# EAST-J/Dynhor

Hardware: AMD Instinct MI355X
Metric: training rays/sec (higher is better)
Workload: dtype f32; 1 GPU; custom_shoes-shaped synthetic seq, 512x512, 2048 rays x (64+64) samples per rank, NeuS SDF(8x256, skip 4, softplus100) + colour(4x256) MLP, full training iteration; family=neus, frames=64, rays_per_rank=2048, samples_per_ray=128, parallelism=dp1, loss=rgb L1 + 0.1 eikonal + 0.1 mask BCE + 0.05 mono-normal

## Files before the change

### dynhor_amd/_lib.py

```python
import ctypes
import os

import torch

_HERE = os.path.dirname(os.path.abspath(__file__))
LIB_PATH = os.path.join(_HERE, "libdynhor_hip.so")
_LIB = None

_vp, _i64, _i32, _f32 = ctypes.c_void_p, ctypes.c_int64, ctypes.c_int, ctypes.c_float

SIGNATURES = {
    "dh_version": (_i32, []),
    "dh_strerror": (ctypes.c_char_p, [_i32]),
    "dh_set_arithmetic": (_i32, [_i32]),
    "dh_get_arithmetic": (_i32, []),
    "dh_hash_set_scatter_mode": (_i32, [_i32]),
    "dh_num_params": (_i64, []),
    "dh_packed_floats": (_i64, []),
    "dh_param_layout": (_i32, [_i32, _i32, ctypes.POINTER(_i64), ctypes.POINTER(_i64), ctypes.POINTER(_i64),
                               ctypes.POINTER(_i32), ctypes.POINTER(_i32)]),
    "dh_packed_section": (_i32, [_i32, ctypes.POINTER(_i64), ctypes.POINTER(_i64)]),
    "dh_pack_weights": (_i32, [_vp, _vp, _vp]),
    "dh_pack_weights_ex": (_i32, [_i32, _vp, _vp, _vp]),
    "dh_sdf_nograd": (_i32, [_vp, _vp, _i64, _vp, _vp]),
    "dh_workspace_floats": (_i32, [_i64, ctypes.POINTER(_i64), ctypes.POINTER(_i64), ctypes.POINTER(_i64)]),
    "dh_range_words": (_i32, [ctypes.POINTER(_i64), ctypes.POINTER(_i64), ctypes.POINTER(_f32)]),
    "dh_mlp_forward": (_i32, [_vp, _vp, _vp, _i32, _i64, _vp, _vp, _vp, _vp, _vp]),
    "dh_sdf_forward": (_i32, [_vp, _vp, _i64, _vp, _vp, _vp]),
    "dh_sdf_gradient": (_i32, [_vp, _vp, _i64, _vp, _vp, _i32, _vp]),
    "dh_color_forward": (_i32, [_vp, _vp, _vp, _i32, _vp, _i64, _vp, _vp, _i32, _vp]),
    "dh_color_backward": (_i32, [_vp, _vp, _vp, _i64, _vp, _vp, _vp]),
    "dh_sdf_tangent": (_i32, [_vp, _vp, _vp, _i64, _vp, _vp]),
    "dh_sdf_backward": (_i32, [_vp, _vp, _i64, _vp, _vp]),
    "dh_color_backward_rays": (_i32, [_vp, _vp, _vp, _vp, _i32, _i64, _vp, _vp, _vp, _vp, _vp]),
    "dh_sdf_backward_rays": (_i32, [_vp, _vp, _vp, _vp, _i64, _vp, _vp, _vp]),
    "dh_weight_grads_gemm": (_i32, [_i64, _vp, _vp]),
    "dh_weight_grads_fold": (_i32, [_vp, _vp, _i64, _vp, _vp, _vp]),
    "dh_mlp_backward": (_i32, [_vp, _vp, _vp, _i64] + [_vp] * 7),
    "dh_sdf_nograd_ex": (_i32, [_i32, _vp, _vp, _i64, _vp, _vp]),
    "dh_mlp_forward_ex": (_i32, [_i32, _vp, _vp, _vp, _i32, _i64, _vp, _vp, _vp, _vp, _vp]),
    "dh_sdf_forward_ex": (_i32, [_i32, _vp, _vp, _i64, _vp, _vp, _vp]),
    "dh_sdf_gradient_ex": (_i32, [_i32, _vp, _vp, _i64, _vp, _vp, _i32, _vp]),
    "dh_color_forward_ex": (_i32, [_i32, _vp, _vp, _vp, _i32, _vp, _i64, _vp, _vp, _i32, _vp]),
    "dh_color_backward_ex": (_i32, [_i32, _vp, _vp, _vp, _i64, _vp, _vp, _vp]),
    "dh_sdf_tangent_ex": (_i32, [_i32, _vp, _vp, _vp, _i64, _vp, _vp]),
    "dh_sdf_backward_ex": (_i32, [_i32, _vp, _vp, _i64, _vp, _vp]),
    "dh_color_backward_rays_ex": (_i32, [_i32, _vp, _vp, _vp, _vp, _i32, _i64, _vp, _vp, _vp, _vp, _vp]),
    "dh_sdf_backward_rays_ex": (_i32, [_i32, _vp, _vp, _vp, _vp, _i64, _vp, _vp, _vp]),
    "dh_weight_grads_gemm_ex": (_i32, [_i32, _i64, _vp, _vp]),
    "dh_mlp_backward_ex": (_i32, [_i32, _vp, _vp, _vp, _i64] + [_vp] * 7),
    "dh_adam_step": (_i32, [_vp, _vp, _vp, _vp, _i64, _f32, _f32, _f32, _f32, _i64, _f32, _vp]),
    "dh_hashgrid_entries": (_i64, []),
    "dh_hashgrid_level": (_i32, [_i32, ctypes.POINTER(_f32), ctypes.POINTER(ctypes.c_uint32), ctypes.POINTER(ctypes.c_uint32),
                                 ctypes.POINTER(ctypes.c_uint32)]),
    "dh_hashgrid_encode": (_i32, [_vp, _vp, _i64, _vp, _vp]),
    "dh_hashgrid_encode_backward": (_i32, [_vp, _vp, _i64, _vp, _vp]),
    "dh_hash_num_params": (_i64, []),
    "dh_hash_packed_floats": (_i64, []),
    "dh_hash_param_layout": (_i32, [_i32, _i32, ctypes.POINTER(_i64), ctypes.POINTER(_i64), ctypes.POINTER(_i64),
                                    ctypes.POINTER(_i32), ctypes.POINTER(_i32)]),
    "dh_hash_pack_weights": (_i32, [_vp, _vp, _vp]),
    "dh_hash_workspace_floats": (_i32, [_i64, ctypes.POINTER(_i64), ctypes.POINTER(_i64)]),
    "dh_hash_sdf_nograd": (_i32, [_vp, _vp, _vp, _i64, _f32, _vp, _vp]),
    "dh_hash_geo_forward": (_i32, [_vp, _vp, _vp, _i64, _f32, _f32, _vp, _i32, _vp, _vp, _vp, _vp, _vp]),
    "dh_hash_color_forward": (_i32, [_vp, _vp, _vp, _vp, _i32, _i64, _vp, _vp, _vp]),
    "dh_hash_color_backward": (_i32, [_vp, _vp, _vp, _vp, _vp, _i32, _i64, _vp, _vp, _vp, _vp, _vp]),
    "dh_hash_geo_backward": (_i32, [_vp, _vp, _vp, _vp, _vp, _vp, _i64, _f32, _f32, _vp, _vp, _vp]),
    "dh_hash_weight_grads": (_i32, [_vp, _vp, _i64, _vp, _vp, _vp, _vp]),
    "dh_hash_weight_grads_parts": (_i32, [_vp, _vp, _i64, _vp, _vp, _vp, _i32, _vp]),
    "dh_gen_rays": (_i32, [_vp] * 6 + [_i32, _i32, _i32, _i32, _vp, _vp, _i64, _vp, _vp, _vp, _vp]),
    "dh_coarse_samples": (_i32, [_vp] * 5 + [_i64, _i32, _vp, _vp, _vp]),
    "dh_upsample_step": (_i32, [_vp] * 4 + [_i64, _i32, _i32, _f32, _vp, _vp, _vp]),
    "dh_merge_samples": (_i32, [_vp] * 4 + [_i64, _i32, _i32, _vp, _vp, _vp]),
    "dh_midpoints": (_i32, [_vp] * 3 + [_i64, _i32, _f32, _vp, _vp]),
    "dh_render_scan_fwd": (_i32, [_vp] * 7 + [_f32, _f32, _vp, _i64, _i32] + [_vp] * 9),
    "dh_render_scan_bwd": (_i32, [_vp] * 7 + [_f32, _f32, _vp, _i64, _i32] + [_vp] * 11),
    "dh_render_scan_bwd_rays": (_i32, [_vp] * 7 + [_f32, _f32, _vp, _i64, _i32] + [_vp] * 12),
    "dh_march_count": (_i32, [_vp] * 6 + [_i32, _f32, _f32, _f32, _i32, _i64, _vp, _vp]),
    "dh_march_emit": (_i32, [_vp] * 6 + [_i32, _f32, _f32, _f32, _i32, _i64] + [_vp] * 7),
    "dh_trace_init": (_i32, [_vp] * 3 + [_i32, _i32, _i32, _i32, _f32] + [_vp] * 6),
    "dh_trace_step": (_i32, [_vp] * 5 + [_i64, _i64] + [_vp] * 10 + [_f32, _f32, _f32, _f32, _i32, _i64, _vp, _vp]),
    "dh_trace_points": (_i32, [_vp] * 4 + [_i64, _i64, _i64, _vp, _vp]),
    "dh_trace_compact": (_i32, [_vp] * 6 + [_i64, _i64, _i64] + [_vp] * 5),
    "dh_trace_compose": (_i32, [_vp] * 6 + [_i64, _vp, _i32, _i32, _i32, _i32, _i32, _vp, _vp, _i32] + [_vp] * 5),
    "dh_render_scan_fwd_packed": (_i32, [_vp] * 7 + [_f32, _f32, _vp, _i64] + [_vp] * 11),
    "dh_render_scan_bwd_packed": (_i32, [_vp] * 7 + [_f32, _f32, _vp, _i64] + [_vp] * 13),
    "dh_neus_loss": (_i32, [_vp] * 6 + [_i64, _f32, _f32, _f32] + [_vp] * 6),
    "dh_corr_loss": (_i32, [_vp] * 7 + [_i32, _vp, _i64, _i32, _f32, _f32, _f32, _vp, _vp, _vp, _vp, _vp]),
    "dh_nearest_sqdist_workspace": (_i64, [_i64, _i64]),
    "dh_nearest_sqdist": (_i32, [_vp, _i64, _vp, _i64, _vp, _vp, _vp, _vp]),
    "dh_mesh_sdf_record_floats": (_i32, []),
    "dh_mesh_sdf_prepare": (_i32, [_vp, _i64, _vp, _i64, _vp, _vp]),
    "dh_mesh_sdf_query_workspace": (_i64, [_i64, _i64]),
    "dh_mesh_sdf_query": (_i32, [_vp, _i64, _vp, _i64, _vp, _vp, _vp, _vp, _vp]),
    "dh_icp_correspond_workspace": (_i64, [_i64, _i64, _i64]),
    "dh_icp_correspond": (_i32, [_vp, _i64, _vp, _i64, _vp, _i64, _vp, _vp, _vp, _vp]),
    "dh_icp_moments_sums": (_i32, [_i32]),
    "dh_icp_moments_workspace": (_i64, [_i64, _i64, _i32]),
    "dh_icp_moments": (_i32, [_vp] * 9 + [_i64, _i64, _i64, _vp, _vp, _vp]),
    "dh_label_dilate": (_i32, [_vp, _i64, _i32, _i32, _i32, _vp, _vp, _vp]),
    "dh_mesh_mask_votes": (_i32, [_vp, _i64, _vp, _vp, _vp, _vp, _i64, _i32, _i32, _vp, _vp, _vp]),
    "dh_mesh_components": (_i32, [_vp, _i64, _i64, _vp, _vp]),
    "dh_hull_accumulate": (_i32, [_vp, _i64, _vp, _vp, _vp, _vp, _i64, _i32, _i32, _i32, _i32, _vp, _vp, _vp, _vp]),
    "dh_mesh_raster_depth": (_i32, [_vp, _i64, _vp, _i64, _vp, _vp, _vp, _i64, _i32, _i32, _vp, _vp]),
    "dh_mesh_bake_colors": (_i32, [_vp, _vp, _i64, _vp, _vp, _vp, _vp, _vp, _vp, _i64, _i32, _i32, _f32, _f32, _vp, _vp, _vp]),
    "dh_mesh_shade": (_i32, [_vp, _vp, _vp, _i64, _vp, _i64, _vp, _vp, _vp, _vp, _i64, _i32, _i32, _vp, _vp, _f32, _vp, _vp, _vp]),
    "dh_texture_bake": (_i32, [_vp, _vp, _i64, _vp, _i64, _vp, _vp, _i32, _vp, _vp, _vp, _vp, _vp, _vp, _i64, _i32, _i32, _f32, _f32, _i32,
                               _vp, _vp, _vp]),
    "dh_mesh_shade_tex": (_i32, [_vp, _vp, _i64, _vp, _i64, _vp, _vp, _i32, _i32, _vp, _vp, _vp, _vp, _i64, _i32, _i32, _vp, _vp, _f32,
                                 _i32, _vp, _vp, _vp]),
    "dh_label_edt": (_i32, [_vp, _i64, _i32, _i32, _i32, _i32, _vp, _vp, _vp]),
    "dh_sil_nearest_workspace": (_i64, [_i64, _i32, _i32]),
    "dh_sil_nearest": (_i32, [_vp, _i64, _vp, _i64, _vp, _vp, _vp, _i64, _i32, _i32, _f32, _vp, _vp, _vp]),
    "dh_sil_loss_sums": (_i32, []),
    "dh_sil_loss_grad_workspace": (_i64, [_i64, _i32, _i32]),
    "dh_sil_loss_grad": (_i32, [_vp, _vp, _i64, _vp, _i64] + [_vp] * 6 + [_i64, _i32, _i32, _f32, _f32, _f32, _vp, _vp, _vp]),
    "dh_image_blur": (_i32, [_vp, _vp, _i64, _i32, _i32, _vp, _i32, _vp, _vp, _vp]),
    "dh_photo_loss_sums": (_i32, []),
    "dh_photo_loss_grad_workspace": (_i64, [_i64, _i64]),
    "dh_photo_loss_grad": (_i32, [_vp, _vp, _vp, _i64, _vp, _vp, _vp, _vp, _vp, _i64, _i32, _i32, _f32, _f32, _f32, _f32, _vp, _vp, _vp]),
    "dh_match_gray": (_i32, [_vp, _i64, _i32, _i32, _f32, _vp, _vp, _vp]),
    "dh_match_search": (_i32, [_vp, _vp, _i64, _i32, _i32, _vp, _i64, _i32, _i32, _i32, _i64, _vp, _vp, _vp]),
    "dh_ssim_sums": (_i32, []),
    "dh_ssim_workspace": (_i64, [_i64, _i32, _i32]),
    "dh_ssim": (_i32, [_vp, _vp, _vp, _i64, _i32, _i32, ctypes.POINTER(_i32), _i32, ctypes.c_uint64, _vp, _vp, _vp, _vp]),
    "dh_label_boxes": (_i32, [_vp, _i64, _i32, _i32, _vp, _vp]),
    "dh_sil_crop_pack": (_i32, [_vp, _i64, _i32, _i32, _vp, _i32, _vp, _vp, _vp]),
    "dh_sil_bank_score": (_i32, [_vp, _vp, _i64, _vp, _i64, _i32, _vp, _vp]),
    "dh_mc_block_points": (_i32, [_vp, _vp, _vp, _i32, _vp, _i64, _i32, _vp, _vp]),
    "dh_mc_count": (_i32, [_vp, _vp, _i64, _i32, _i32, _f32, _vp, _vp, _vp, _vp, _vp, _vp]),
    "dh_mc_emit": (_i32, [_vp, _vp, _i64, _i32, _i32, _f32, _vp, _vp, _i64, _vp, _vp, _vp]),
    "dh_simplify_grid": (_i32, [ctypes.POINTER(_f32), ctypes.POINTER(_f32), _i64, ctypes.POINTER(_f32), ctypes.POINTER(_i32)]),
    "dh_simplify_cells": (_i32, [_vp, _i64, ctypes.POINTER(_f32), _f32, ctypes.POINTER(_i32), _vp, _vp]),
    "dh_simplify_sums": (_i32, []),
    "dh_simplify_quadrics": (_i32, [_vp, _i64, _vp, _i64, _vp, _vp, _vp, _i64, ctypes.POINTER(_f32), _f32, ctypes.POINTER(_i32),
                                    ctypes.c_double, _i32, _vp, _vp, _vp, _vp]),
    "dh_simplify_faces": (_i32, [_vp, _i64, _vp, _i64, _i64, _vp, _vp, _vp, _vp]),
}


class DynhorHipError(RuntimeError):
    pass


def lib():
    global _LIB
    if _LIB is None:
        if not os.path.exists(LIB_PATH):
            raise DynhorHipError(
                f"{LIB_PATH} not found: the HIP extension is mandatory (no CPU fallback). "
                "Build it with: python -c 'import __graft_entry__ as g; g.build()'")
        L = ctypes.CDLL(LIB_PATH)
        for name, (res, args) in SIGNATURES.items():
            fn = getattr(L, name)
            fn.restype = res
            fn.argtypes = args
        _LIB = L
# ... 96 lines not shown
```

### dynhor_amd/csrc/api.hip

```cpp
#include "../../include/dynhor_hip.h"
#include "kernels.h"
#include "hash_layout.h"
#include "layout.h"
#include "workspace.h"

using namespace dh;

namespace dh {
static int g_arith = DH_ARITH_SPLIT_F16;
static int g_hash_scatter = 0;
int hash_scatter_mode() { return __atomic_load_n(&g_hash_scatter, __ATOMIC_RELAXED); }
}

namespace {
inline bool misaligned16(const void* p) { return (reinterpret_cast<uintptr_t>(p) & 15u) != 0; }
inline bool bad_arith(int a) { return a != DH_ARITH_SPLIT_BF16 && a != DH_ARITH_FP32_MFMA && a != DH_ARITH_SPLIT_F16; }
inline bool bad_arith_form(int a) {
    const int form = a & ~0xff;
    return bad_arith(a & 0xff) || (form != 0 && form != DH_CHAIN_FORM_TILE && form != DH_CHAIN_FORM_PAIR) ||
           (form != 0 && (a & 0xff) != DH_ARITH_SPLIT_F16);
}
inline int cur_arith() { return __atomic_load_n(&dh::g_arith, __ATOMIC_RELAXED); }
#ifndef DH_GRID_DIV
#define DH_GRID_DIV 1
#endif
constexpr int DEFAULT_GRID = 256 * 2 / DH_GRID_DIV;
}

extern "C" {

int dh_version(void) { return 3; }

int dh_set_arithmetic(int mode) {
    if (bad_arith(mode)) return DH_ERR_BAD_ARG;
    __atomic_store_n(&dh::g_arith, mode, __ATOMIC_RELAXED);
    return DH_OK;
}
int dh_get_arithmetic(void) { return __atomic_load_n(&dh::g_arith, __ATOMIC_RELAXED); }

int dh_hash_set_scatter_mode(int mode) {
    if (mode < 0 || mode > 2) return DH_ERR_BAD_ARG;
    __atomic_store_n(&dh::g_hash_scatter, mode, __ATOMIC_RELAXED);
    return DH_OK;
}

const char* dh_strerror(int status) {
    switch (status) {
        case DH_OK: return "ok";
        case DH_ERR_BAD_ARG: return "bad argument (null / negative size / misaligned pointer)";
        case DH_ERR_UNSUPPORTED: return "unsupported configuration";
        case DH_ERR_LAUNCH: return "kernel launch failed (hipGetLastError)";
        default: return "unknown dynhor_hip status";
    }
}

int64_t dh_num_params(void) { return N_PARAMS; }
int64_t dh_packed_floats(void) { return PACKH.total; }

int dh_packed_section(int section, int64_t* offset_floats, int64_t* n_floats) {
    if (!offset_floats || !n_floats) return DH_ERR_BAD_ARG;
    switch (section) {
        case 0: *offset_floats = PACKT.stream; *n_floats = PACKT_STREAM_FLOATS; break;
        case 1: *offset_floats = PACKT.bias10; *n_floats = 10 * 256; break;
        case 2: *offset_floats = PACKH.stream; *n_floats = PACKTH_STREAM_FLOATS; break;
        case 3: *offset_floats = PACKH.bias11; *n_floats = 11 * 256; break;
        case 4: *offset_floats = PACKH.wabs; *n_floats = 16; break;
        default: return DH_ERR_BAD_ARG;
    }
    return DH_OK;
}

int dh_param_layout(int net, int layer, int64_t* bias_off, int64_t* g_off, int64_t* v_off, int* out_dim, int* in_dim) {
    if (!bias_off || !g_off || !v_off || !out_dim || !in_dim) return DH_ERR_BAD_ARG;
    if (net == 0) {
        if (layer < 0 || layer >= N_SDF) return DH_ERR_BAD_ARG;
        const LinOff o = sdf_off(layer);
        *bias_off = o.bias; *g_off = o.g; *v_off = o.v; *out_dim = SDF_DIMS[layer].out; *in_dim = SDF_DIMS[layer].in;
    } else if (net == 1) {
        *bias_off = *g_off = *v_off = VARIANCE_OFF; *out_dim = 1; *in_dim = 1;
    } else if (net == 2) {
        if (layer < 0 || layer >= N_COL) return DH_ERR_BAD_ARG;
        const LinOff o = col_off(layer);
        *bias_off = o.bias; *g_off = o.g; *v_off = o.v; *out_dim = COL_DIMS[layer].out; *in_dim = COL_DIMS[layer].in;
    } else {
        return DH_ERR_BAD_ARG;
    }
    return DH_OK;
}

int dh_pack_weights(const float* params, float* packed, void* stream) {
    if (!params || !packed || misaligned16(packed)) return DH_ERR_BAD_ARG;
    return launch_pack_weights(params, packed, 7, static_cast<hipStream_t>(stream));
}
int dh_pack_weights_ex(int arithmetic, const float* params, float* packed, void* stream) {
    if (!params || !packed || misaligned16(packed) || bad_arith(arithmetic)) return DH_ERR_BAD_ARG;
    return launch_pack_weights(params, packed, 1 << arithmetic, static_cast<hipStream_t>(stream));
}

// ... 138 lines not shown
int dh_sdf_forward(const float* packed, const float* pts, int64_t npts, float* ws, float* sdf, void* stream) {
    return dh_sdf_forward_ex(cur_arith(), packed, pts, npts, ws, sdf, stream);
}
int dh_sdf_gradient(const float* packed, const float* pts, int64_t npts, float* ws, float* normals, int save, void* stream) {
    return dh_sdf_gradient_ex(cur_arith(), packed, pts, npts, ws, normals, save, stream);
}
int dh_color_forward(const float* packed, const float* pts, const float* dirs, int n_per_ray, const float* normals,
                     int64_t npts, float* ws, float* color, int save, void* stream) {
    return dh_color_forward_ex(cur_arith(), packed, pts, dirs, n_per_ray, normals, npts, ws, color, save, stream);
}
int dh_mlp_forward(const float* packed, const float* pts, const float* dirs, int n_per_ray, int64_t npts, float* ws,
                   float* sdf, float* normals, float* color, void* stream) {
    return dh_mlp_forward_ex(cur_arith(), packed, pts, dirs, n_per_ray, npts, ws, sdf, normals, color, stream);
}
int dh_color_backward(const float* packed, const float* colors, const float* d_colors, int64_t npts, float* ws,
                      float* d_normals, void* stream) {
    return dh_color_backward_ex(cur_arith(), packed, colors, d_colors, npts, ws, d_normals, stream);
}
int dh_sdf_tangent(const float* packed, const float* pts, const float* d_normals, int64_t npts, float* ws, void* stream) {
    return dh_sdf_tangent_ex(cur_arith(), packed, pts, d_normals, npts, ws, stream);
}
int dh_sdf_backward(const float* packed, const float* d_sdf, int64_t npts, float* ws, void* stream) {
    return dh_sdf_backward_ex(cur_arith(), packed, d_sdf, npts, ws, stream);
}
int dh_color_backward_rays(const float* packed, const float* colors, const float* d_colors, const float* dirs, int n_per_ray,
                           int64_t npts, float* ws, float* d_normals, float* d_pts, float* d_dirs_pts, void* stream) {
    return dh_color_backward_rays_ex(cur_arith(), packed, colors, d_colors, dirs, n_per_ray, npts, ws, d_normals, d_pts, d_dirs_pts, stream);
}
int dh_sdf_backward_rays(const float* packed, const float* d_sdf, const float* pts, const float* d_normals, int64_t npts,
                         float* ws, float* d_pts, void* stream) {
    return dh_sdf_backward_rays_ex(cur_arith(), packed, d_sdf, pts, d_normals, npts, ws, d_pts, stream);
}
int dh_weight_grads_gemm(int64_t npts, float* ws, void* stream) { return dh_weight_grads_gemm_ex(cur_arith(), npts, ws, stream); }
int dh_mlp_backward(const float* packed, const float* params, const float* pts, int64_t npts, float* ws,
                    const float* colors, const float* d_sdf, float* d_normals, const float* d_colors, float* grad_flat,
                    void* stream) {
    return dh_mlp_backward_ex(cur_arith(), packed, params, pts, npts, ws, colors, d_sdf, d_normals, d_colors, grad_flat, stream);
}

int dh_gen_rays(const uint8_t* rgb, const int8_t* label, const uint8_t* normal, const float* R, const float* T,
                const float* Kinv, int H, int W, int n_frames, int frame, const int64_t* px, const int64_t* py, int64_t B,
                float* rays, float* near, float* far, void* stream) {
    if (B < 0 || H <= 0 || W <= 0 || frame < 0 || frame >= n_frames) return DH_ERR_BAD_ARG;
    if (B == 0) return DH_OK;
    if (!rgb || !label || !normal || !R || !T || !Kinv || !px || !py || !rays || !near || !far) return DH_ERR_BAD_ARG;
    return launch_gen_rays(rgb, label, normal, R, T, Kinv, H, W, frame, px, py, B, rays, near, far, static_cast<hipStream_t>(stream));
}

int dh_coarse_samples(const float* rays_o, const float* rays_d, const float* near, const float* far, const float* t_rand,
                      int64_t B, int n_samples, float* z, float* pts, void* stream) {
    if (B < 0 || n_samples <= 0) return DH_ERR_BAD_ARG;
    if (B == 0) return DH_OK;
    if (!rays_o || !rays_d || !near || !far || !z || !pts) return DH_ERR_BAD_ARG;
    return launch_coarse_samples(rays_o, rays_d, near, far, t_rand, B, n_samples, z, pts, static_cast<hipStream_t>(stream));
}

int dh_upsample_step(const float* rays_o, const float* rays_d, const float* z, const float* sdf, int64_t B, int n_cur,
                     int n_new, float inv_s, float* z_new, float* pts_new, void* stream) {
    if (B < 0 || n_cur < 2 || n_new <= 0) return DH_ERR_BAD_ARG;
    if (n_cur > 128 || n_new > 64) return DH_ERR_UNSUPPORTED;
    if (B == 0) return DH_OK;
    if (!rays_o || !rays_d || !z || !sdf || !z_new || !pts_new) return DH_ERR_BAD_ARG;
    return launch_upsample(rays_o, rays_d, z, sdf, B, n_cur, n_new, inv_s, z_new, pts_new, static_cast<hipStream_t>(stream));
}

int dh_merge_samples(const float* z, const float* z_new, const float* sdf, const float* sdf_new, int64_t B, int n_cur,
                     int n_new, float* z_out, float* sdf_out, void* stream) {
    if (B < 0 || n_cur <= 0 || n_new <= 0) return DH_ERR_BAD_ARG;
    if (n_cur > 128 || n_new > 64) return DH_ERR_UNSUPPORTED;
    if (B == 0) return DH_OK;
    if (!z || !z_new || !z_out) return DH_ERR_BAD_ARG;
    if (sdf_out && (!sdf || !sdf_new)) return DH_ERR_BAD_ARG;
    return launch_merge(z, z_new, sdf, sdf_new, B, n_cur, n_new, z_out, sdf_out, static_cast<hipStream_t>(stream));
}

int dh_midpoints(const float* rays_o, const float* rays_d, const float* z, int64_t B, int n, float sample_dist, float* pts,
                 void* stream) {
    if (B < 0 || n <= 0) return DH_ERR_BAD_ARG;
    if (B == 0) return DH_OK;
    if (!rays_o || !rays_d || !z || !pts) return DH_ERR_BAD_ARG;
    return launch_midpoints(rays_o, rays_d, z, B, n, sample_dist, pts, static_cast<hipStream_t>(stream));
}

int dh_render_scan_fwd(const float* rays_o, const float* rays_d, const float* z, const float* sdf, const float* normals,
                       const float* colors, const float* inv_s, float cos_anneal_ratio, float sample_dist,
                       const float* background_rgb, int64_t B, int n, float* weights, float* color, float* weight_sum,
                       float* weight_max, float* cdf, float* inside_sphere, float* eik_partial, float* normal_map,
                       void* stream) {
    if (B < 0 || n <= 0) return DH_ERR_BAD_ARG;
    if (n > 128) return DH_ERR_UNSUPPORTED;
    if (B == 0) return DH_OK;
    if (!rays_o || !rays_d || !z || !sdf || !normals || !colors || !inv_s || !weights || !color || !weight_sum ||
        !weight_max || !cdf || !inside_sphere || !eik_partial) return DH_ERR_BAD_ARG;
    return launch_render_fwd(rays_o, rays_d, z, sdf, normals, colors, inv_s, cos_anneal_ratio, sample_dist, background_rgb,
                             B, n, weights, color, weight_sum, weight_max, cdf, inside_sphere, eik_partial, normal_map,
                             nullptr, nullptr, static_cast<hipStream_t>(stream));
}

int dh_render_scan_bwd(const float* rays_o, const float* rays_d, const float* z, const float* sdf, const float* normals,
                       const float* colors, const float* inv_s, float cos_anneal_ratio, float sample_dist,
                       const float* background_rgb, int64_t B, int n, const float* d_color, const float* d_weight_sum,
                       const float* d_weights, const float* d_gradients, const float* d_normal_map, const float* eik_coef,
                       float* d_sdf, float* d_normals, float* d_colors, float* d_inv_s, void* stream) {
    if (B < 0 || n <= 0) return DH_ERR_BAD_ARG;
    if (n > 128) return DH_ERR_UNSUPPORTED;
    if (B == 0) return DH_OK;
    if (!rays_o || !rays_d || !z || !sdf || !normals || !colors || !inv_s || !d_color || !eik_coef || !d_sdf ||
        !d_normals || !d_colors || !d_inv_s) return DH_ERR_BAD_ARG;
    return launch_render_bwd(rays_o, rays_d, z, sdf, normals, colors, inv_s, cos_anneal_ratio, sample_dist, background_rgb,
                             B, n, d_color, d_weight_sum, d_weights, d_gradients, d_normal_map, eik_coef, d_sdf, d_normals, d_colors,
                             d_inv_s, nullptr, nullptr, nullptr, static_cast<hipStream_t>(stream));
}

int dh_render_scan_bwd_rays(const float* rays_o, const float* rays_d, const float* z, const float* sdf, const float* normals,
                            const float* colors, const float* inv_s, float cos_anneal_ratio, float sample_dist,
                            const float* background_rgb, int64_t B, int n, const float* d_color, const float* d_weight_sum,
                            const float* d_weights, const float* d_gradients, const float* d_normal_map, const float* eik_coef,
                            float* d_sdf, float* d_normals, float* d_colors, float* d_inv_s, float* d_rays_d, void* stream) {
    if (B < 0 || n <= 0) return DH_ERR_BAD_ARG;
    if (n > 128) return DH_ERR_UNSUPPORTED;
    if (B == 0) return DH_OK;
    if (!rays_o || !rays_d || !z || !sdf || !normals || !colors || !inv_s || !d_color || !eik_coef || !d_sdf ||
        !d_normals || !d_colors || !d_inv_s || !d_rays_d) return DH_ERR_BAD_ARG;
    return launch_render_bwd(rays_o, rays_d, z, sdf, normals, colors, inv_s, cos_anneal_ratio, sample_dist, background_rgb,
                             B, n, d_color, d_weight_sum, d_weights, d_gradients, d_normal_map, eik_coef, d_sdf, d_normals, d_colors,
                             d_inv_s, d_rays_d, nullptr, nullptr, static_cast<hipStream_t>(stream));
}

int dh_march_count(const float* rays_o, const float* rays_d, const float* near, const float* far, const float* u,
                   const uint8_t* occupancy, int res, float radius, float step, float half_step, int max_samples, int64_t B,
                   int32_t* cnt, void* stream) {
    if (B < 0 || res <= 0 || !(radius > 0.f) || !(step > 0.f) || max_samples <= 0) return DH_ERR_BAD_ARG;
    if (max_samples > 1024) return DH_ERR_UNSUPPORTED;
    if (B == 0) return DH_OK;
    if (!rays_o || !rays_d || !near || !far || !occupancy || !cnt) return DH_ERR_BAD_ARG;
    return launch_march_count(rays_o, rays_d, near, far, u, occupancy, res, radius, step, half_step, max_samples, B, cnt,
                              static_cast<hipStream_t>(stream));
}

int dh_march_emit(const float* rays_o, const float* rays_d, const float* near, const float* far, const float* u,
                  const uint8_t* occupancy, int res, float radius, float step, float half_step, int max_samples, int64_t B,
                  const int64_t* off, const int32_t* keep, float* t_start, float* pts, float* dirs_pts, int32_t* ray_idx,
                  void* stream) {
    if (B < 0 || res <= 0 || !(radius > 0.f) || !(step > 0.f) || max_samples <= 0) return DH_ERR_BAD_ARG;
    if (max_samples > 1024) return DH_ERR_UNSUPPORTED;
    if (B == 0) return DH_OK;
    if (!rays_o || !rays_d || !near || !far || !occupancy || !off || !t_start || !pts || !dirs_pts || !ray_idx) return DH_ERR_BAD_ARG;
    return launch_march_emit(rays_o, rays_d, near, far, u, occupancy, res, radius, step, half_step, max_samples, B, off, keep,
                             t_start, pts, dirs_pts, ray_idx, static_cast<hipStream_t>(stream));
}

int dh_render_scan_fwd_packed(const float* rays_o, const float* rays_d, const float* t_start, const float* sdf, const float* normals,
                              const float* colors, const float* inv_s, float cos_anneal_ratio, float step,
                              const float* background_rgb, int64_t B, const int64_t* seg_off, const int32_t* seg_cnt,
                              float* weights, float* color, float* weight_sum, float* weight_max, float* cdf,
                              float* inside_sphere, float* eik_partial, float* normal_map, void* stream) {
    if (B < 0) return DH_ERR_BAD_ARG;
    if (B == 0) return DH_OK;
    if (!rays_o || !rays_d || !t_start || !sdf || !normals || !colors || !inv_s || !seg_off || !seg_cnt || !weights || !color ||
        !weight_sum || !weight_max || !cdf || !inside_sphere || !eik_partial) return DH_ERR_BAD_ARG;
    return launch_render_fwd(rays_o, rays_d, t_start, sdf, normals, colors, inv_s, cos_anneal_ratio, step, background_rgb, B, 0,
                             weights, color, weight_sum, weight_max, cdf, inside_sphere, eik_partial, normal_map, seg_off, seg_cnt,
                             static_cast<hipStream_t>(stream));
}

int dh_render_scan_bwd_packed(const float* rays_o, const float* rays_d, const float* t_start, const float* sdf, const float* normals,
                              const float* colors, const float* inv_s, float cos_anneal_ratio, float step,
                              const float* background_rgb, int64_t B, const int64_t* seg_off, const int32_t* seg_cnt,
                              const float* d_color, const float* d_weight_sum, const float* d_weights, const float* d_gradients,
                              const float* d_normal_map, const float* eik_coef, float* d_sdf, float* d_normals, float* d_colors,
                              float* d_inv_s, void* stream) {
    if (B < 0) return DH_ERR_BAD_ARG;
    if (B == 0) return DH_OK;
    if (!rays_o || !rays_d || !t_start || !sdf || !normals || !colors || !inv_s || !seg_off || !seg_cnt || !d_color || !eik_coef ||
        !d_sdf || !d_normals || !d_colors || !d_inv_s) return DH_ERR_BAD_ARG;
    return launch_render_bwd(rays_o, rays_d, t_start, sdf, normals, colors, inv_s, cos_anneal_ratio, step, background_rgb, B, 0,
                             d_color, d_weight_sum, d_weights, d_gradients, d_normal_map, eik_coef, d_sdf, d_normals, d_colors,
                             d_inv_s, nullptr, seg_off, seg_cnt, static_cast<hipStream_t>(stream));
}

int dh_adam_step(float* params, const float* grad, float* exp_avg, float* exp_avg_sq, int64_t n, float lr, float beta1,
                 float beta2, float eps, int64_t step, float grad_scale, void* stream) {
    if (n < 0 || step < 1) return DH_ERR_BAD_ARG;
    if (n == 0) return DH_OK;
    if (!params || !grad || !exp_avg || !exp_avg_sq) return DH_ERR_BAD_ARG;
    return launch_adam(params, grad, exp_avg, exp_avg_sq, n, lr, beta1, beta2, eps, step, grad_scale,
                       static_cast<hipStream_t>(stream));
}

int dh_neus_loss(const float* color, const float* weight_sum, const float* normal_map, const float* eik_partial,
                 const float* rays, const float* R, int64_t B, float igr_weight, float mask_weight, float normal_weight,
                 float* stats, float* d_color, float* d_weight_sum, float* d_normal_map, float* eik_coef, void* stream) {
    if (B <= 0) return DH_ERR_BAD_ARG;
    if (!color || !weight_sum || !eik_partial || !rays || !stats || !d_color || !d_weight_sum || !eik_coef)
        return DH_ERR_BAD_ARG;
    if (normal_weight > 0.f && (!normal_map || !R || !d_normal_map)) return DH_ERR_BAD_ARG;
    return launch_loss(color, weight_sum, normal_map, eik_partial, rays, R, B, igr_weight, mask_weight, normal_weight, stats,
                       d_color, d_weight_sum, d_normal_map, eik_coef, static_cast<hipStream_t>(stream));
}

int dh_corr_loss(const float* rays_o, const float* rays_d, const float* z, const float* weights, const float* corr,
                 const float* R_all, const float* T_all, int n_frames, const float* K, int64_t B, int n, float sample_dist,
                 float delta_px, float corr_weight, float* stats, float* residual_px, float* d_weights, float* pose_adjoints,
                 void* stream) {
    if (B <= 0 || n <= 0 || n_frames <= 0 || !(delta_px > 0.f)) return DH_ERR_BAD_ARG;
    if (!rays_o || !rays_d || !z || !weights || !corr || !R_all || !T_all || !K || !stats || !residual_px || !d_weights)
        return DH_ERR_BAD_ARG;
    return launch_corr_loss(rays_o, rays_d, z, weights, corr, R_all, T_all, n_frames, K, B, n, sample_dist, delta_px, corr_weight,
                            stats, residual_px, d_weights, pose_adjoints, static_cast<hipStream_t>(stream));
}

int64_t dh_hashgrid_entries(void) { return hashgrid_entries(); }

int dh_hashgrid_level(int level, float* scale, uint32_t* resolution, uint32_t* offset, uint32_t* dense) {
    if (!scale || !resolution || !offset || !dense) return DH_ERR_BAD_ARG;
    return hashgrid_level(level, scale, resolution, offset, dense) ? DH_ERR_BAD_ARG : DH_OK;
}

int dh_hashgrid_encode(const float* table, const float* x01, int64_t n, float* out, void* stream) {
    if (n < 0) return DH_ERR_BAD_ARG;
    if (n == 0) return DH_OK;
    if (!table || !x01 || !out || (reinterpret_cast<uintptr_t>(table) & 7u) || (reinterpret_cast<uintptr_t>(out) & 7u))
        return DH_ERR_BAD_ARG;
    return launch_hashgrid_fwd(table, x01, n, out, static_cast<hipStream_t>(stream));
}

int dh_hashgrid_encode_backward(const float* x01, const float* d_out, int64_t n, float* d_table, void* stream) {
    if (n < 0) return DH_ERR_BAD_ARG;
    if (n == 0) return DH_OK;
    if (!x01 || !d_out || !d_table || (reinterpret_cast<uintptr_t>(d_out) & 7u)) return DH_ERR_BAD_ARG;
    return launch_hashgrid_bwd(x01, d_out, n, d_table, static_cast<hipStream_t>(stream));
}

int64_t dh_hash_num_params(void) { return hash_num_params(); }
int64_t dh_hash_packed_floats(void) { return HP_TOTAL; }

int dh_hash_param_layout(int net, int layer, int64_t* bias_off, int64_t* g_off, int64_t* v_off, int* out_dim, int* in_dim) {
    if (!bias_off || !g_off || !v_off || !out_dim || !in_dim) return DH_ERR_BAD_ARG;
    const HashParamOff P = make_hash_param_off(hashgrid_entries());
    if (net == 0 && layer == 0) { *bias_off = P.g0_b; *g_off = P.g0_g; *v_off = P.g0_v; *out_dim = 64; *in_dim = HM_GIN; }
    else if (net == 0 && layer == 1) { *bias_off = P.g1_b; *g_off = P.g1_g; *v_off = P.g1_v; *out_dim = HM_GOUT; *in_dim = 64; }
    else if (net == 1 && layer == 0) { *bias_off = *g_off = *v_off = P.variance; *out_dim = 1; *in_dim = 1; }
    else if (net == 2 && layer == 0) { *bias_off = P.c0_b; *g_off = P.c0_g; *v_off = P.c0_v; *out_dim = 64; *in_dim = HM_CIN; }
    else if (net == 2 && layer == 1) { *bias_off = P.c1_b; *g_off = P.c1_g; *v_off = P.c1_v; *out_dim = 64; *in_dim = 64; }
    else if (net == 2 && layer == 2) { *bias_off = P.c2_b; *g_off = P.c2_g; *v_off = P.c2_v; *out_dim = 3; *in_dim = 64; }
    else if (net == 3 && layer == 0) { *bias_off = *g_off = *v_off = P.table; *out_dim = (int)hashgrid_entries(); *in_dim = 2; }
    else return DH_ERR_BAD_ARG;
    return DH_OK;
}

int dh_hash_pack_weights(const float* params, float* packed, void* stream) {
    if (!params || !packed) return DH_ERR_BAD_ARG;
    return launch_hash_pack(params, packed, static_cast<hipStream_t>(stream));
}

int dh_hash_workspace_floats(int64_t npts, int64_t* infer_floats, int64_t* total_floats) {
    if (npts < 0 || !infer_floats || !total_floats) return DH_ERR_BAD_ARG;
    *infer_floats = hash_infer_workspace_floats(npts);
    *total_floats = hash_workspace_floats(npts);
    return DH_OK;
}

static inline bool al16(const void* p) { return (reinterpret_cast<uintptr_t>(p) & 15u) == 0; }

int dh_hash_sdf_nograd(const float* params, const float* packed, const float* pts, int64_t n, float radius, float* sdf,
                       void* stream) {
    if (n < 0 || !(radius > 0.f)) return DH_ERR_BAD_ARG;
    if (n == 0) return DH_OK;
    if (!params || !packed || !pts || !sdf || !al16(params) || !al16(packed)) return DH_ERR_BAD_ARG;
    return launch_hash_sdf_nograd(params, packed, pts, n, radius, sdf, static_cast<hipStream_t>(stream));
// ... 588 lines not shown
```

### dynhor_amd/csrc/kernels.h

```cpp
#pragma once
#include <hip/hip_runtime.h>
#include <stdint.h>
#include "layout.h"

namespace dh {

enum : int { ARITH_BF16 = 0, ARITH_FP32 = 1, ARITH_F16 = 2 };
int hash_scatter_mode();

int launch_pack_weights(const float* params, float* packed, int arith_mask, hipStream_t stream);

inline int ok() { return hipGetLastError() == hipSuccess ? 0 : -3; }
inline int grid_for(int64_t npts, int grid) {
    const int64_t ntiles = (npts + TM - 1) / TM;
    return (int)(ntiles < grid ? ntiles : grid);
}

int launch_sdf_nograd(const float* packed, const float* pts, int64_t npts, float* sdf, int grid, int arith, hipStream_t stream);
int launch_sdf_nograd_t(const float* packed, const float* pts, int64_t npts, float* sdf, bool h2, hipStream_t stream);
int launch_sdf_fwd_train_t(const float* packed, const float* pts, int64_t npts, float* sdf, float* feat, float* act, float* eaux,
                           unsigned* absmax, bool h2, hipStream_t stream);

int launch_sdf_fwd_train(const float* packed, const float* pts, int64_t npts, float* sdf, float* feat, float* act,
                         float* eaux, float* absmax, int grid, int arith, hipStream_t stream);
int launch_sdf_grad(const float* packed, const float* pts, int64_t npts, const float* act, float* asave, float* normals,
                    int save, float* gesave, float* absmax, int grid, int arith, hipStream_t stream);
int launch_color_fwd(const float* packed, const float* pts, const float* dirs, int n_per_ray, const float* normals,
                     const float* feat, int64_t npts, float* color, float* cact, float* caux, int save, float* absmax, int grid,
                     int arith, hipStream_t stream);
int launch_sdf_grad_h(const float* packed, const float* pts, int64_t npts, const float* act, float* asave, float* normals,
                      int save, float* gesave, unsigned* absmax, int grid, hipStream_t stream);
int launch_color_fwd_h(const float* packed, const float* pts, const float* dirs, int n_per_ray, const float* normals,
                       const float* feat, int64_t npts, float* color, float* cact, float* caux, int save, unsigned* absmax,
                       int grid, hipStream_t stream);
int launch_color_bwd_h(const float* packed, const float* colors, const float* d_colors, const float* dirs, int n_per_ray,
                       int64_t npts, const float* cact, float* czbar, float* featbar, float* d_normals, float* tpart,
                       float* d_pts, float* d_dirs_pts, unsigned* absmax, unsigned* tmax, int grid, hipStream_t st);
int launch_sdf_tangent_h(const float* packed, const float* pts, const float* d_normals, int64_t npts, const float* act,
                         const float* asave, float* t0aux, float* tsave, float* rsave, float* tpart, unsigned* absmax, unsigned* tmax,
                         int grid, hipStream_t st);
int launch_sdf_bwd_h(const float* packed, const float* d_sdf, const float* pts, const float* d_normals, int64_t npts,
                     const float* act, const float* rsave, const float* featbar, const float* gesave, float* zbar, float* tpart,
                     float* d_pts, unsigned* absmax, unsigned* tmax, int grid, hipStream_t st);

enum : int { CHAIN_FORM_AUTO = 0, CHAIN_FORM_TILE = 1, CHAIN_FORM_PAIR = 2 };
bool pair_form_available();
int pair_form_cus();
inline bool use_pair_form(int form, int64_t npts, bool auto_pair) {
    if (form == CHAIN_FORM_PAIR) return true;
    if (form == CHAIN_FORM_TILE || !auto_pair) return false;
    const int cus = pair_form_cus();
    return cus > 0 && (npts + TM - 1) / TM >= 2 * (int64_t)cus;
}
int launch_color_fwd_p(const float* packed, const float* pts, const float* dirs, int n_per_ray, const float* normals,
                       const float* feat, int64_t npts, float* color, float* cact, float* caux, int save, unsigned* absmax,
                       hipStream_t stream);

int launch_sdf_grad_p(const float* packed, const float* pts, int64_t npts, const float* act, float* asave, float* normals, int save,
                      float* gesave, unsigned* absmax, hipStream_t stream);

int launch_color_bwd_p(const float* packed, const float* colors, const float* d_colors, int64_t npts, const float* cact, float* czbar,
                       float* featbar, float* d_normals, float* tpart, unsigned* absmax, unsigned* tmax, hipStream_t stream);

int launch_gen_rays(const uint8_t* rgb, const int8_t* label, const uint8_t* normal, const float* R, const float* T,
                    const float* Kinv, int H, int W, int frame, const int64_t* px, const int64_t* py, int64_t B,
                    float* rays, float* near, float* far, hipStream_t st);
int launch_coarse_samples(const float* o, const float* d, const float* near, const float* far, const float* t_rand,
                          int64_t B, int n, float* z, float* pts, hipStream_t st);
int launch_upsample(const float* o, const float* d, const float* z, const float* sdf, int64_t B, int n, int n_new,
                    float inv_s, float* z_new, float* pts_new, hipStream_t st);
int launch_merge(const float* z, const float* z_new, const float* sdf, const float* sdf_new, int64_t B, int n, int n_new,
                 float* z_out, float* sdf_out, hipStream_t st);
int launch_midpoints(const float* o, const float* d, const float* z, int64_t B, int n, float sample_dist, float* pts,
                     hipStream_t st);
int launch_render_fwd(const float* o, const float* d, const float* z, const float* sdf, const float* normals,
                      const float* colors, const float* inv_s, float car, float sample_dist, const float* bg, int64_t B,
                      int n, float* weights, float* color, float* wsum, float* wmax, float* cdf, float* inside, float* eik,
                      float* nmap, const int64_t* seg_off, const int32_t* seg_cnt, hipStream_t st);
int launch_render_bwd(const float* o, const float* d, const float* z, const float* sdf, const float* normals,
                      const float* colors, const float* inv_s, float car, float sample_dist, const float* bg, int64_t B,
                      int n, const float* d_color, const float* d_wsum, const float* d_weights, const float* d_gradients,
                      const float* d_nmap, const float* eik_coef, float* d_sdf, float* d_normals, float* d_colors,
                      float* d_inv_s, float* d_rays_d, const int64_t* seg_off, const int32_t* seg_cnt, hipStream_t st);
int launch_march_count(const float* o, const float* d, const float* near, const float* far, const float* u, const uint8_t* occ,
                       int res, float radius, float step, float half_step, int max_samples, int64_t B, int32_t* cnt,
                       hipStream_t st);
int launch_march_emit(const float* o, const float* d, const float* near, const float* far, const float* u, const uint8_t* occ,
                      int res, float radius, float step, float half_step, int max_samples, int64_t B, const int64_t* off,
                      const int32_t* keep, float* t_start, float* pts, float* dirs_pts, int32_t* ray_idx, hipStream_t st);
int launch_trace_init(const float* R, const float* T, const float* Kinv, int h, int w, int level, float bound, int64_t N, float* o,
                      float* d, float* t, float* t_far, uint8_t* state, hipStream_t st);
int launch_trace_step(const int32_t* idx, const int32_t* count, const float* s, const float* o, const float* d, int64_t rays_per_view,
                      int64_t N, float* t, const float* t_far, float* t_lo, float* s_lo, float* t_hi, float* s_hi, uint8_t* state,
                      uint16_t* nq, uint8_t* nref, uint8_t* flags, float eps, float relax, float min_step, float max_step,
                      int refine_steps, int64_t n_max, float* pts, hipStream_t st);
int launch_trace_points(const int32_t* idx, const float* o, const float* d, const float* t, int64_t rays_per_view, int64_t N, int64_t n,
                        float* pts, hipStream_t st);
int launch_trace_compact(const int32_t* idx, const int32_t* count, const uint8_t* state, const float* o, const float* d, const float* t,
                         int64_t rays_per_view, int64_t N, int64_t n_max, int32_t* block_off, int32_t* idx_out, int32_t* count_out,
                         float* pts_out, hipStream_t st);
int launch_trace_compose(const uint8_t* state, const float* t, const float* d, const int32_t* slot, const float* normals,
                         const float* colors, int64_t n_hits, const float* R, int h, int w, int level, int H, int W, int background,
                         const uint8_t* frame_rgb, const int32_t* frame_idx, int n_frames, int64_t N, uint8_t* rgb, float* depth,
                         uint8_t* normal, uint8_t* hit, hipStream_t st);
int launch_loss(const float* color, const float* wsum, const float* nmap, const float* eik, const float* rays,
                const float* R, int64_t B, float igr_w, float mask_w, float normal_w, float* stats, float* d_color,
                float* d_wsum, float* d_nmap, float* eik_coef, hipStream_t st);

int launch_corr_loss(const float* rays_o, const float* rays_d, const float* z, const float* weights, const float* corr,
                     const float* R_all, const float* T_all, int n_frames, const float* K, int64_t B, int n, float sample_dist,
                     float delta_px, float corr_w, float* stats, float* residual_px, float* d_weights, float* pose_adj,
                     hipStream_t st);

int launch_color_bwd(const float* packed, const float* colors, const float* d_colors, int64_t npts, const float* cact,
                     float* czbar, float* featbar, float* d_normals, float* tpart, float* absmax, int grid, int arith, hipStream_t st);
int launch_color_bwd_rays(const float* packed, const float* colors, const float* d_colors, const float* dirs, int n_per_ray,
                          int64_t npts, const float* cact, float* czbar, float* featbar, float* d_normals, float* tpart,
                          float* d_pts, float* d_dirs_pts, float* absmax, int grid, int arith, hipStream_t st);
int launch_sdf_bwd_rays(const float* packed, const float* d_sdf, const float* pts, const float* d_normals, int64_t npts,
                        const float* act, const float* rsave, const float* featbar, const float* gesave, float* zbar,
                        float* tpart, float* d_pts, float* absmax, int grid, int arith, hipStream_t st);
int launch_sdf_tangent(const float* packed, const float* pts, const float* d_normals, int64_t npts, const float* act,
                       const float* asave, float* t0aux, float* tsave, float* rsave, float* tpart, float* absmax, int grid, int arith,
                       hipStream_t st);
int launch_sdf_bwd(const float* packed, const float* d_sdf, int64_t npts, const float* act, const float* rsave,
                   const float* featbar, float* zbar, float* tpart, float* absmax, int grid, int arith, hipStream_t st);
struct Workspace;
int launch_weight_grads_gemm(const Workspace& w, float* slabs, float* tred, int G, int nS, int arith, hipStream_t st);
int launch_weight_grads_fold(const Workspace& w, float* slabs, float* tred, int G, int nS, const float* params,
                             const float* packed, float* grad, hipStream_t st);

int launch_adam(float* p, const float* g, float* m, float* v, int64_t n, float lr, float b1, float b2, float eps,
                int64_t step, float grad_scale, hipStream_t st);

int64_t hashgrid_entries();
int hashgrid_level(int l, float* scale, uint32_t* res, uint32_t* offset, uint32_t* dense);
int launch_hashgrid_fwd(const float* table, const float* x01, int64_t n, float* out, hipStream_t st);
int launch_hashgrid_bwd(const float* x01, const float* d_out, int64_t n, float* d_table, hipStream_t st);

int64_t hash_num_params();
int64_t hash_workspace_floats(int64_t n);
int launch_hash_pack(const float* params, float* hp, hipStream_t st);
int launch_hash_sdf_nograd(const float* params, const float* hp, const float* pts, int64_t n, float radius, float* sdf,
                           hipStream_t st);
int64_t hash_infer_workspace_floats(int64_t n);
int launch_hash_geo_fwd(const float* params, const float* hp, const float* pts, int64_t n, float radius, float eps,
                        float* ws, int save, float* sdf, float* feat, float* grad, const int64_t* n_act, hipStream_t st);
int launch_sh_color_fwd(const float* hp, const float* feat, const float* normals, const float* dirs, int n_per_ray,
                        int64_t n, float* color, const int64_t* n_act, hipStream_t st);
int launch_sh_color_bwd(const float* hp, const float* feat, const float* normals, const float* dirs, const float* d_color,
                        int n_per_ray, int64_t n, float* ws, float* d_feat, float* d_normals, const int64_t* n_act, hipStream_t st);
int launch_hash_geo_bwd(const float* params, const float* hp, const float* pts, const float* d_sdf, const float* d_feat,
                        const float* d_grad, int64_t n, float radius, float eps, float* ws, const int64_t* n_act, hipStream_t st);
int launch_hash_weight_grads(const float* params, const float* hp, int64_t n, float* ws, float* grad, const int64_t* n_act,
                             int parts, hipStream_t st);

int64_t nearest_sqdist_workspace(int64_t nq, int64_t nr);
int launch_nearest_sqdist(const float* q, int64_t nq, const float* ref, int64_t nr, float* d2, int32_t* idx, void* ws, hipStream_t st);

int mesh_sdf_record_floats();
int64_t mesh_sdf_query_workspace(int64_t n, int64_t nf);
int64_t mesh_sdf_max_faces();
int launch_mesh_sdf_prepare(const float* verts, int64_t nv, const int32_t* faces, int64_t nf, float* rec, hipStream_t st);
int launch_mesh_sdf_query(const float* rec, int64_t nf, const float* pts, int64_t n, float* sqdist, int32_t* face, float* wind, void* ws,
                          hipStream_t st);

int64_t icp_correspond_workspace(int64_t n, int64_t m, int64_t h);
int launch_icp_correspond(const float* src, int64_t n, const float* tgt, int64_t m, const float* xf, int64_t h, float* d2, int32_t* idx,
                          void* ws, hipStream_t st);
int icp_moments_sums(int plane);
int64_t icp_moments_workspace(int64_t n, int64_t h, int plane);
int launch_icp_moments(const float* src, const float* tgt, const float* nrm, const float* xf, const int32_t* idx, const float* d2,
                       const float* thr, const float* osrc, const float* otgt, int64_t n, int64_t m, int64_t h, double* out, void* ws,
                       hipStream_t st);

int launch_sum64_reduce(const double* partial, int64_t groups, int blocks, int K, double* out, hipStream_t st);

int launch_label_dilate(const int8_t* label, int64_t n_frames, int H, int W, int radius, uint8_t* tmp, uint8_t* keep, hipStream_t st);
int launch_mesh_mask_votes(const float* verts, int64_t nv, const uint8_t* keep, const float* R, const float* T, const float* K,
                           int64_t n_frames, int H, int W, int32_t* bg_votes, int32_t* seen, hipStream_t st);
int launch_mesh_components(const int64_t* faces, int64_t nf, int64_t nv, int32_t* labels, hipStream_t st);

int launch_hull_accumulate(const float* pts, int64_t n, const float* sd, const float* R, const float* T, const float* K, int n_frames,
                           int H, int W, int frame0, int m, float* topk, int32_t* arg, int32_t* seen, hipStream_t st);

int launch_mesh_raster_depth(const float* verts, int64_t nv, const int64_t* faces, int64_t nf, const float* R, const float* T,
                             const float* K, int64_t n_frames, int H, int W, uint64_t* zbuf, hipStream_t st);
int launch_mesh_bake_colors(const float* verts, const float* normals, int64_t nv, const uint8_t* rgb, const uint8_t* usable,
                            const uint64_t* zbuf, const float* R, const float* T, const float* K, int64_t n_frames, int H, int W,
                            float depth_eps, float min_cos, float* acc, int32_t* n_views, hipStream_t st);
int launch_mesh_shade(const float* verts, const float* normals, const uint8_t* colors, int64_t nv, const int64_t* faces, int64_t nf,
                      const uint64_t* zbuf, const float* R, const float* T, const float* K, int64_t n_frames, int H, int W,
                      const uint8_t* rgb, const int8_t* label, float alpha, uint8_t* out, int64_t* counts, hipStream_t st);
int launch_texture_bake(const float* verts, const float* normals, int64_t nv, const int64_t* faces, int64_t nf, const float* uv,
                        const int32_t* owner, int S, const uint8_t* rgb, const uint8_t* usable, const uint64_t* zbuf, const float* R,
                        const float* T, const float* K, int64_t n_frames, int H, int W, float depth_eps, float min_cos, int sharpen,
                        float* acc, int32_t* n_views, hipStream_t st);
int64_t shade_tex_blocks_per_frame(int H, int W);
int launch_mesh_shade_tex(const float* verts, const float* normals, int64_t nv, const int64_t* faces, int64_t nf, const float* uv,
                          const uint8_t* tex, int Sh, int Sw, const uint64_t* zbuf, const float* R, const float* T, const float* K,
                          int64_t n_frames, int H, int W, const uint8_t* rgb, const uint8_t* usable, float alpha, int lit, uint8_t* out,
                          int64_t* sums, hipStream_t st);

int launch_label_edt(const int8_t* label, int64_t n_frames, int H, int W, int value, int rmax, float* tmp, float* out, hipStream_t st);
int64_t sil_nearest_workspace(int64_t n_frames, int H, int W);
int launch_sil_nearest(const float* verts, int64_t nv, const int64_t* faces, int64_t nf, const float* R, const float* T, const float* K,
                       int64_t n_frames, int H, int W, float rmax_px, uint64_t* near, void* ws, hipStream_t st);
int sil_loss_sums();
int64_t sil_loss_grad_workspace(int64_t n_frames, int H, int W);
int launch_sil_loss_grad(const uint64_t* near, const float* verts, int64_t nv, const int64_t* faces, int64_t nf, const float* R,
                         const float* T, const float* K, const float* d2_obj, const float* d2_hand, const int8_t* label, int64_t n_frames,
                         int H, int W, float sigma, float cut, float edge_offset, double* out, void* ws, hipStream_t st);

int image_blur_max_radius();
int launch_image_blur(const uint8_t* rgb, const uint8_t* usable, int64_t n_frames, int H, int W, const float* taps, int radius,
                      float* tmp, float* out, hipStream_t st);
// ... 48 lines not shown
```

### dynhor_amd/csrc/kernels_ray.hip

```cpp
#include "tile.h"
#include "kernels.h"

namespace dh {

__device__ __forceinline__ float wave_sum(float v) {
    DH_UNROLL for (int off = 32; off > 0; off >>= 1) v += __shfl_xor(v, off);
    return v;
}
__device__ __forceinline__ float wave_max(float v) {
    DH_UNROLL for (int off = 32; off > 0; off >>= 1) v = fmaxf(v, __shfl_xor(v, off));
    return v;
}
__device__ __forceinline__ float wave_excl_prod(float v, int lane) {
    float x = v;
    DH_UNROLL for (int off = 1; off < 64; off <<= 1) {
        const float y = __shfl_up(x, off);
        if (lane >= off) x *= y;
    }
    const float e = __shfl_up(x, 1);
    return lane == 0 ? 1.f : e;
}
__device__ __forceinline__ float wave_incl_sum(float v, int lane) {
    float x = v;
    DH_UNROLL for (int off = 1; off < 64; off <<= 1) {
        const float y = __shfl_up(x, off);
        if (lane >= off) x += y;
    }
    return x;
}
__device__ __forceinline__ float wave_excl_suffix_sum(float v, int lane) {
    float x = v;
    DH_UNROLL for (int off = 1; off < 64; off <<= 1) {
        const float y = __shfl_down(x, off);
        if (lane + off < 64) x += y;
    }
    const float e = __shfl_down(x, 1);
    return lane == 63 ? 0.f : e;
}
__device__ __forceinline__ float sigmoidf(float x) { return 1.f / (1.f + __expf(-x)); }

__global__ __launch_bounds__(256) void gen_rays_kernel(const uint8_t* __restrict__ rgb, const int8_t* __restrict__ label,
                                                       const uint8_t* __restrict__ normal, const float* __restrict__ R,
                                                       const float* __restrict__ T, const float* __restrict__ Kinv,
                                                       int H, int W, int frame, const int64_t* __restrict__ px,
                                                       const int64_t* __restrict__ py, int64_t B, float* __restrict__ rays,
                                                       float* __restrict__ near, float* __restrict__ far) {
    const int64_t i = (int64_t)blockIdx.x * 256 + threadIdx.x;
    if (i >= B) return;
    const int64_t x = px[i], y = py[i];
    const float u = (float)x, v = (float)y;
    float p[3], dcam[3];
    DH_UNROLL for (int r = 0; r < 3; ++r) p[r] = Kinv[r * 3 + 0] * u + Kinv[r * 3 + 1] * v + Kinv[r * 3 + 2];
    const float inv = 1.f / sqrtf(p[0] * p[0] + p[1] * p[1] + p[2] * p[2]);
    DH_UNROLL for (int r = 0; r < 3; ++r) dcam[r] = p[r] * inv;
    const float* Rf = R + (int64_t)frame * 9;
    const float* Tf = T + (int64_t)frame * 3;
    float o[3], d[3];
    DH_UNROLL for (int c = 0; c < 3; ++c) {
        d[c] = Rf[0 * 3 + c] * dcam[0] + Rf[1 * 3 + c] * dcam[1] + Rf[2 * 3 + c] * dcam[2];
        o[c] = -(Rf[0 * 3 + c] * Tf[0] + Rf[1 * 3 + c] * Tf[1] + Rf[2 * 3 + c] * Tf[2]);
    }
    const int64_t pix = ((int64_t)frame * H + y) * W + x;
    float* out = rays + i * 14;
    DH_UNROLL for (int c = 0; c < 3; ++c) { out[c] = o[c]; out[3 + c] = d[c]; }
    DH_UNROLL for (int c = 0; c < 3; ++c) out[6 + c] = (float)rgb[pix * 3 + c] / 255.0f;
    const int lab = (int)label[pix];
    out[9] = lab > 0 ? 1.f : 0.f;
    out[10] = lab >= 0 ? 1.f : 0.f;
    DH_UNROLL for (int c = 0; c < 3; ++c) out[11 + c] = (float)normal[pix * 3 + c] / 255.0f * 2.0f - 1.0f;
    const float a = d[0] * d[0] + d[1] * d[1] + d[2] * d[2];
    const float b = 2.f * (o[0] * d[0] + o[1] * d[1] + o[2] * d[2]);
    const float mid = 0.5f * (-b) / a;
    near[i] = mid - 1.f;
    far[i] = mid + 1.f;
}

__global__ __launch_bounds__(256) void coarse_samples_kernel(const float* __restrict__ rays_o, const float* __restrict__ rays_d,
                                                             const float* __restrict__ near, const float* __restrict__ far,
                                                             const float* __restrict__ t_rand, int64_t B, int n,
                                                             float* __restrict__ z, float* __restrict__ pts) {
    const int64_t i = (int64_t)blockIdx.x * 256 + threadIdx.x;
    if (i >= B * n) return;
    const int64_t b = i / n;
    const int j = (int)(i - b * n);
    const float lin = (n > 1) ? (float)j / (float)(n - 1) : 0.f;
    float zz = near[b] + (far[b] - near[b]) * lin;
    if (t_rand) zz += (t_rand[b] - 0.5f) * 2.0f / (float)n;
    z[i] = zz;
    DH_UNROLL for (int c = 0; c < 3; ++c) pts[i * 3 + c] = rays_o[b * 3 + c] + rays_d[b * 3 + c] * zz;
}

__global__ __launch_bounds__(256) void upsample_kernel(const float* __restrict__ rays_o, const float* __restrict__ rays_d,
                                                       const float* __restrict__ z, const float* __restrict__ sdf,
                                                       int64_t B, int n, int n_new, float inv_s,
                                                       float* __restrict__ z_new, float* __restrict__ pts_new) {
    __shared__ float s_cdf[4][132];
    __shared__ float s_z[4][132];
    const int wave = threadIdx.x >> 6, lane = threadIdx.x & 63;
    const int64_t ray = (int64_t)blockIdx.x * 4 + wave;
    if (ray >= B) return;
    const float ox = rays_o[ray * 3], oy = rays_o[ray * 3 + 1], oz = rays_o[ray * 3 + 2];
    const float dx = rays_d[ray * 3], dy = rays_d[ray * 3 + 1], dz = rays_d[ray * 3 + 2];
    const int e0 = 2 * lane, e1 = e0 + 1;
    const float* zr = z + ray * n;
    const float* sr = sdf + ray * n;
    const float z0 = e0 < n ? zr[e0] : 0.f, z1 = e1 < n ? zr[e1] : 0.f;
    const float f0 = e0 < n ? sr[e0] : 0.f, f1 = e1 < n ? sr[e1] : 0.f;
    auto radius = [&](float t) {
        const float x = ox + dx * t, y = oy + dy * t, w = oz + dz * t;
        return sqrtf(x * x + y * y + w * w);
    };
    const float r0 = radius(z0), r1 = radius(z1);
    const float z2 = __shfl_down(z0, 1), f2 = __shfl_down(f0, 1), r2 = __shfl_down(r0, 1);
    const bool vA = e0 < n - 1, vB = e1 < n - 1;
    const float cosA_raw = (f1 - f0) / (z1 - z0 + 1e-5f);
    const float cosB_raw = (f2 - f1) / (z2 - z1 + 1e-5f);
    float prevA = __shfl_up(cosB_raw, 1);
    if (lane == 0) prevA = 0.f;
    const float insA = ((r0 < 1.f) || (r1 < 1.f)) ? 1.f : 0.f;
    const float insB = ((r1 < 1.f) || (r2 < 1.f)) ? 1.f : 0.f;
    const float cosA = fminf(fmaxf(fminf(prevA, cosA_raw), -1e3f), 0.f) * insA;
    const float cosB = fminf(fmaxf(fminf(cosA_raw, cosB_raw), -1e3f), 0.f) * insB;
    auto alpha_of = [&](float fa, float fb, float za, float zb, float cs) {
        const float mid = (fa + fb) * 0.5f, dist = zb - za;
        const float pe = mid - cs * dist * 0.5f, ne = mid + cs * dist * 0.5f;
        const float pc = sigmoidf(pe * inv_s), nc = sigmoidf(ne * inv_s);
        return (pc - nc + 1e-5f) / (pc + 1e-5f);
    };
    const float aA = vA ? alpha_of(f0, f1, z0, z1, cosA) : 0.f;
    const float aB = vB ? alpha_of(f1, f2, z1, z2, cosB) : 0.f;
    const float tA = 1.f - aA + 1e-7f, tB = 1.f - aB + 1e-7f;
    const float excl = wave_excl_prod(tA * tB, lane);
    const float wA = vA ? aA * excl + 1e-5f : 0.f;
    const float wB = vB ? aB * excl * tA + 1e-5f : 0.f;
    const float tot = wave_sum(wA + wB);
    const float pA = wA / tot, pB = wB / tot;
    const float incl = wave_incl_sum(pA + pB, lane);
    float* cdf = s_cdf[wave];
    float* zs = s_z[wave];
    if (lane == 0) cdf[0] = 0.f;
    if (vA) cdf[e0 + 1] = incl - pB;
    if (vB) cdf[e1 + 1] = incl;
    if (e0 < n) zs[e0] = z0;
    if (e1 < n) zs[e1] = z1;
    __builtin_amdgcn_fence(__ATOMIC_RELEASE, "workgroup");
    __builtin_amdgcn_wave_barrier();
    __builtin_amdgcn_fence(__ATOMIC_ACQUIRE, "workgroup");
    if (lane < n_new) {
        const float u = (0.5f + (float)lane) / (float)n_new;
        int lo = 0, hi = n;
        while (lo < hi) {
            const int mid = (lo + hi) >> 1;
            if (cdf[mid] <= u) lo = mid + 1; else hi = mid;
        }
        const int below = max(lo - 1, 0), above = min(lo, n - 1);
        const float c0 = cdf[below], c1 = cdf[above];
        float denom = c1 - c0;
        if (denom < 1e-5f) denom = 1.f;
        const float t = (u - c0) / denom;
        const float b0 = zs[below], b1 = zs[above];
        const float zn = b0 + t * (b1 - b0);
        z_new[ray * n_new + lane] = zn;
        float* pp = pts_new + (ray * n_new + lane) * 3;
        pp[0] = ox + dx * zn; pp[1] = oy + dy * zn; pp[2] = oz + dz * zn;
    }
}

__global__ __launch_bounds__(256) void merge_kernel(const float* __restrict__ z, const float* __restrict__ z_new,
                                                    const float* __restrict__ sdf, const float* __restrict__ sdf_new,
                                                    int64_t B, int n, int n_new, float* __restrict__ z_out,
                                                    float* __restrict__ sdf_out) {
    const int wave = threadIdx.x >> 6, lane = threadIdx.x & 63;
    const int64_t ray = (int64_t)blockIdx.x * 4 + wave;
    if (ray >= B) return;
    const int e0 = 2 * lane, e1 = e0 + 1;
    const float INF = __builtin_inff();
    const float z0 = e0 < n ? z[ray * n + e0] : INF, z1 = e1 < n ? z[ray * n + e1] : INF;
    const float zn = lane < n_new ? z_new[ray * n_new + lane] : INF;
    int c0 = 0, c1 = 0, cn = 0;
    for (int k = 0; k < n_new; ++k) {
        const float v = __shfl(zn, k);
        c0 += (v < z0) ? 1 : 0;
        c1 += (v < z1) ? 1 : 0;
    }
    for (int k = 0; k < n_new; ++k) {
        const float v = __shfl(zn, k);
        const int cnt = __popcll(__ballot(z0 <= v)) + __popcll(__ballot(z1 <= v));
        if (lane == k) cn = cnt;
    }
    const int no = n + n_new;
    float* zo = z_out + ray * no;
    if (e0 < n) zo[e0 + c0] = z0;
    if (e1 < n) zo[e1 + c1] = z1;
    if (lane < n_new) zo[lane + cn] = zn;
    if (sdf_out) {
        float* so = sdf_out + ray * no;
        if (e0 < n) so[e0 + c0] = sdf[ray * n + e0];
        if (e1 < n) so[e1 + c1] = sdf[ray * n + e1];
        if (lane < n_new) so[lane + cn] = sdf_new[ray * n_new + lane];
    }
}

__global__ __launch_bounds__(256) void midpoints_kernel(const float* __restrict__ rays_o, const float* __restrict__ rays_d,
                                                        const float* __restrict__ z, int64_t B, int n, float sample_dist,
                                                        float* __restrict__ pts) {
    const int64_t i = (int64_t)blockIdx.x * 256 + threadIdx.x;
    if (i >= B * n) return;
    const int64_t b = i / n;
    const int j = (int)(i - b * n);
    const float dist = (j + 1 < n) ? z[i + 1] - z[i] : sample_dist;
    const float mid = z[i] + dist * 0.5f;
    DH_UNROLL for (int c = 0; c < 3; ++c) pts[i * 3 + c] = rays_o[b * 3 + c] + rays_d[b * 3 + c] * mid;
}

struct RenderElem {
    float alpha, alpha_raw, cden, prev, next, ep, en, dist, dtc;
    float relax, nn;
    float n[3], c[3];
};

__device__ __forceinline__ RenderElem render_elem(bool valid, int64_t gp, float zc, float znext, bool last, float sample_dist,
                                                  const float (&o)[3], const float (&d)[3], const float* __restrict__ sdf,
                                                  const float* __restrict__ normals, const float* __restrict__ colors,
                                                  float inv_s, float car, float& inside) {
    RenderElem e{};
    inside = 0.f;
    if (!valid) return e;
    e.dist = last ? sample_dist : znext - zc;
    const float mid = zc + e.dist * 0.5f;
    float pn2 = 0.f;
    DH_UNROLL for (int c = 0; c < 3; ++c) { const float p = o[c] + d[c] * mid; pn2 += p * p; }
    const float pn = sqrtf(pn2);
    inside = pn < 1.0f ? 1.f : 0.f;
    e.relax = pn < 1.2f ? 1.f : 0.f;
    const float s = sdf[gp];
    float tc = 0.f, n2 = 0.f;
    DH_UNROLL for (int c = 0; c < 3; ++c) {
        e.n[c] = normals[gp * 3 + c];
        e.c[c] = colors[gp * 3 + c];
        tc += d[c] * e.n[c];
        n2 += e.n[c] * e.n[c];
    }
    e.nn = sqrtf(n2);
    const float a1 = -tc * 0.5f + 0.5f, a2 = -tc;
    const float ic = -(fmaxf(a1, 0.f) * (1.f - car) + fmaxf(a2, 0.f) * car);
    e.dtc = (a1 > 0.f ? 0.5f * (1.f - car) : 0.f) + (a2 > 0.f ? car : 0.f);
    e.en = s + ic * e.dist * 0.5f;
    e.ep = s - ic * e.dist * 0.5f;
    e.prev = sigmoidf(e.ep * inv_s);
    e.next = sigmoidf(e.en * inv_s);
    e.cden = e.prev + 1e-5f;
    e.alpha_raw = (e.prev - e.next + 1e-5f) / e.cden;
    e.alpha = fminf(fmaxf(e.alpha_raw, 0.f), 1.f);
    return e;
}

constexpr int RENDER_MAX_CHUNKS = 8;
__global__ __launch_bounds__(256) void render_fwd_kernel(const float* __restrict__ rays_o, const float* __restrict__ rays_d,
                                                         const float* __restrict__ z, const float* __restrict__ sdf,
                                                         const float* __restrict__ normals, const float* __restrict__ colors,
                                                         const float* __restrict__ inv_s_p, float car, float sample_dist,
                                                         const float* __restrict__ bg_rgb, int64_t B, int n,
                                                         float* __restrict__ weights, float* __restrict__ color_out,
                                                         float* __restrict__ wsum_out, float* __restrict__ wmax_out,
                                                         float* __restrict__ cdf_out, float* __restrict__ inside_out,
                                                         float* __restrict__ eik_out, float* __restrict__ nmap_out,
                                                         const int64_t* __restrict__ seg_off, const int32_t* __restrict__ seg_cnt) {
    const int wave = threadIdx.x >> 6, lane = threadIdx.x & 63;
    const int64_t ray = (int64_t)blockIdx.x * 4 + wave;
    if (ray >= B) return;
    const float inv_s = inv_s_p[0];
    float o[3], d[3];
    DH_UNROLL for (int c = 0; c < 3; ++c) { o[c] = rays_o[ray * 3 + c]; d[c] = rays_d[ray * 3 + c]; }
    const bool packed = seg_off != nullptr;
    const int64_t rb = packed ? seg_off[ray] : ray * n;
    if (packed) n = min(seg_cnt[ray], 128 * RENDER_MAX_CHUNKS);
    float T_in = 1.f, ws = 0.f, wm = 0.f, en = 0.f, ed = 0.f;
    float col[3] = {0.f, 0.f, 0.f}, nm[3] = {0.f, 0.f, 0.f};
    for (int c0 = 0; c0 == 0 || c0 < n; c0 += 128) {
        const int e0 = c0 + 2 * lane, e1 = e0 + 1;
        const float z0 = e0 < n ? z[rb + e0] : 0.f, z1 = e1 < n ? z[rb + e1] : 0.f;
        float z2 = __shfl_down(z0, 1);
        if (lane == 63) z2 = (e1 + 1 < n) ? z[rb + e1 + 1] : 0.f;
        float in0, in1;
        const RenderElem A = render_elem(e0 < n, rb + e0, z0, z1, packed || e0 == n - 1, sample_dist, o, d, sdf, normals, colors, inv_s, car, in0);
        const RenderElem Bq = render_elem(e1 < n, rb + e1, z1, z2, packed || e1 == n - 1, sample_dist, o, d, sdf, normals, colors, inv_s, car, in1);
        const float tA = (e0 < n) ? 1.f - A.alpha + 1e-7f : 1.f, tB = (e1 < n) ? 1.f - Bq.alpha + 1e-7f : 1.f;
        const float excl = T_in * wave_excl_prod(tA * tB, lane);
        const float w0 = A.alpha * excl, w1 = Bq.alpha * excl * tA;
        ws += wave_sum(w0 + w1);
        wm = fmaxf(wm, wave_max(fmaxf(w0, w1)));
        DH_UNROLL for (int c = 0; c < 3; ++c) col[c] += wave_sum(w0 * A.c[c] + w1 * Bq.c[c]);
        DH_UNROLL for (int c = 0; c < 3; ++c) nm[c] += wave_sum(w0 * A.n[c] + w1 * Bq.n[c]);
        const float g0 = (A.nn - 1.f) * (A.nn - 1.f) * A.relax, g1 = (Bq.nn - 1.f) * (Bq.nn - 1.f) * Bq.relax;
        en += wave_sum(g0 + g1); ed += wave_sum(A.relax + Bq.relax);
// ... 63 lines not shown
            const float excl = T_in * wave_excl_prod(P.tA * P.tB, lane);
            const float q = (P.v0 ? P.wb0 * P.A.alpha * excl : 0.f) + (P.v1 ? P.wb1 * P.Bq.alpha * excl * P.tA : 0.f);
            const float qs = wave_sum(q);
            if (lane == ch) { c_tin = T_in; c_q = qs; }
            T_in = __shfl(excl * P.tA * P.tB, 63);
        }
    }
    float dinv = 0.f;
    float ddir[3] = {0.f, 0.f, 0.f};
    auto elem_bwd = [&](const RenderElem& E, bool valid, float ab, float w, int64_t gp) {
        if (!valid) return;
        const float ar = (E.alpha_raw >= 0.f && E.alpha_raw <= 1.f) ? ab : 0.f;
        const float pb = ar * (1.f - E.alpha_raw) / E.cden;
        const float nb = -ar / E.cden;
        const float xp = pb * E.prev * (1.f - E.prev), xn = nb * E.next * (1.f - E.next);
        d_sdf[gp] = inv_s * (xp + xn);
        const float icb = inv_s * E.dist * 0.5f * (xn - xp);
        dinv += xp * E.ep + xn * E.en;
        const float tcb = icb * E.dtc;
        DH_UNROLL for (int c = 0; c < 3; ++c) ddir[c] += tcb * E.n[c];
        const float ek = (E.nn > 0.f) ? ec * E.relax * 2.f * (E.nn - 1.f) / E.nn : 0.f;
        DH_UNROLL for (int c = 0; c < 3; ++c) {
            float g = tcb * d[c] + ek * E.n[c] + w * dN[c];
            if (d_gradients) g += d_gradients[gp * 3 + c];
            d_normals[gp * 3 + c] = g;
            d_colors[gp * 3 + c] = w * dC[c];
        }
    };
    for (int ch = 0; ch < nchunks; ++ch) {
        const RenderPair P = load_pair(ch * 128);
        float T_in = 1.f, q_after = 0.f;
        if (nchunks > 1) {
            T_in = __shfl(c_tin, ch);
            for (int k = ch + 1; k < nchunks; ++k) q_after += __shfl(c_q, k);
        }
        const float excl = T_in * wave_excl_prod(P.tA * P.tB, lane);
        const float T0 = excl, T1 = excl * P.tA;
        const float w0 = P.A.alpha * T0, w1 = P.Bq.alpha * T1;
        const float q0 = P.v0 ? P.wb0 * w0 : 0.f, q1 = P.v1 ? P.wb1 * w1 : 0.f;
        const float suf = wave_excl_suffix_sum(q0 + q1, lane) + q_after;
        const float ab0 = P.wb0 * T0 - (suf + q1) / P.tA;
        const float ab1 = P.wb1 * T1 - suf / P.tB;
        elem_bwd(P.A, P.v0, ab0, w0, rb + ch * 128 + 2 * lane);
        elem_bwd(P.Bq, P.v1, ab1, w1, rb + ch * 128 + 2 * lane + 1);
    }
    dinv = wave_sum(dinv);
    if (lane == 0) d_inv_s[ray] = dinv;
    if (d_rays_d) {
        DH_UNROLL for (int c = 0; c < 3; ++c) { const float v = wave_sum(ddir[c]); if (lane == 0) d_rays_d[ray * 3 + c] = v; }
    }
}


int launch_gen_rays(const uint8_t* rgb, const int8_t* label, const uint8_t* normal, const float* R, const float* T,
                    const float* Kinv, int H, int W, int frame, const int64_t* px, const int64_t* py, int64_t B,
                    float* rays, float* near, float* far, hipStream_t st) {
    hipLaunchKernelGGL(gen_rays_kernel, dim3((unsigned)((B + 255) / 256)), dim3(256), 0, st, rgb, label, normal, R, T, Kinv,
                       H, W, frame, px, py, B, rays, near, far);
    return ok();
}
int launch_coarse_samples(const float* o, const float* d, const float* near, const float* far, const float* t_rand,
                          int64_t B, int n, float* z, float* pts, hipStream_t st) {
    hipLaunchKernelGGL(coarse_samples_kernel, dim3((unsigned)((B * n + 255) / 256)), dim3(256), 0, st, o, d, near, far, t_rand,
                       B, n, z, pts);
    return ok();
}
int launch_upsample(const float* o, const float* d, const float* z, const float* sdf, int64_t B, int n, int n_new,
                    float inv_s, float* z_new, float* pts_new, hipStream_t st) {
    hipLaunchKernelGGL(upsample_kernel, dim3((unsigned)((B + 3) / 4)), dim3(256), 0, st, o, d, z, sdf, B, n, n_new, inv_s,
                       z_new, pts_new);
    return ok();
}
int launch_merge(const float* z, const float* z_new, const float* sdf, const float* sdf_new, int64_t B, int n, int n_new,
                 float* z_out, float* sdf_out, hipStream_t st) {
    hipLaunchKernelGGL(merge_kernel, dim3((unsigned)((B + 3) / 4)), dim3(256), 0, st, z, z_new, sdf, sdf_new, B, n, n_new,
                       z_out, sdf_out);
    return ok();
}
int launch_midpoints(const float* o, const float* d, const float* z, int64_t B, int n, float sample_dist, float* pts,
                     hipStream_t st) {
    hipLaunchKernelGGL(midpoints_kernel, dim3((unsigned)((B * n + 255) / 256)), dim3(256), 0, st, o, d, z, B, n, sample_dist, pts);
    return ok();
}
int launch_render_fwd(const float* o, const float* d, const float* z, const float* sdf, const float* normals,
                      const float* colors, const float* inv_s, float car, float sample_dist, const float* bg, int64_t B,
                      int n, float* weights, float* color, float* wsum, float* wmax, float* cdf, float* inside, float* eik,
                      float* nmap, const int64_t* seg_off, const int32_t* seg_cnt, hipStream_t st) {
    hipLaunchKernelGGL(render_fwd_kernel, dim3((unsigned)((B + 3) / 4)), dim3(256), 0, st, o, d, z, sdf, normals, colors, inv_s,
                       car, sample_dist, bg, B, n, weights, color, wsum, wmax, cdf, inside, eik, nmap, seg_off, seg_cnt);
    return ok();
}
int launch_render_bwd(const float* o, const float* d, const float* z, const float* sdf, const float* normals,
                      const float* colors, const float* inv_s, float car, float sample_dist, const float* bg, int64_t B,
                      int n, const float* d_color, const float* d_wsum, const float* d_weights, const float* d_gradients,
                      const float* d_nmap, const float* eik_coef, float* d_sdf, float* d_normals, float* d_colors,
                      float* d_inv_s, float* d_rays_d, const int64_t* seg_off, const int32_t* seg_cnt, hipStream_t st) {
    hipLaunchKernelGGL(render_bwd_kernel, dim3((unsigned)((B + 3) / 4)), dim3(256), 0, st, o, d, z, sdf, normals, colors, inv_s,
                       car, sample_dist, bg, B, n, d_color, d_wsum, d_weights, d_gradients, d_nmap, eik_coef, d_sdf, d_normals,
                       d_colors, d_inv_s, d_rays_d, seg_off, seg_cnt);
    return ok();
}

}
```

### dynhor_amd/csrc/optim.hip

```cpp
#include "tile.h"
#include "kernels.h"

namespace dh {

__global__ __launch_bounds__(256) void adam_kernel(float* __restrict__ p, const float* __restrict__ g, float* __restrict__ m,
                                                   float* __restrict__ v, int64_t n, float lr, float b1, float b2, float eps,
                                                   float bc1, float bc2_sqrt, float grad_scale) {
    const int64_t i = (int64_t)blockIdx.x * 256 + threadIdx.x;
    if (i >= n) return;
    const float gi = g[i] * grad_scale;
    const float mi = b1 * m[i] + (1.f - b1) * gi;
    const float vi = b2 * v[i] + (1.f - b2) * gi * gi;
    m[i] = mi;
    v[i] = vi;
    const float denom = sqrtf(vi) / bc2_sqrt + eps;
    p[i] -= (lr / bc1) * (mi / denom);
}

__device__ __forceinline__ float block_sum(float v, float* s_red) {
    DH_UNROLL for (int off = 32; off > 0; off >>= 1) v += __shfl_xor(v, off);
    __syncthreads();
    if ((threadIdx.x & 63) == 0) s_red[threadIdx.x >> 6] = v;
    __syncthreads();
    float t = 0.f;
// ... 79 lines not shown
    const int tid = threadIdx.x;
    const float fx = K[0], fy = K[4], cx = K[2], cy = K[5];
    const float delta = delta_px / fx;
    float a_cv = 0.f, a_l = 0.f, a_r = 0.f;
    for (int64_t b = tid; b < B; b += blockDim.x) {
        const float conf = corr[b * 4 + 2];
        float dt = 0.f;
        float res = 0.f;
        float dy[3] = {0.f, 0.f, 0.f}, dx[3] = {0.f, 0.f, 0.f}, depth_out = 0.f;
        const int j = (int)corr[b * 4 + 3];
        if (conf > 0.f) res = __builtin_inff();
        if (conf > 0.f && j >= 0 && j < n_frames) {
            float depth = 0.f;
            const float* zr = z + b * n;
            const float* wr = weights + b * n;
            for (int k = 0; k < n; ++k) {
                const float dist = (k + 1 < n) ? zr[k + 1] - zr[k] : sample_dist;
                depth = fmaf(wr[k], zr[k] + 0.5f * dist, depth);
            }
            float x[3], y[3], g[3];
            DH_UNROLL for (int c = 0; c < 3; ++c) x[c] = rays_o[b * 3 + c] + depth * rays_d[b * 3 + c];
            const float* Rj = R_all + (int64_t)j * 9;
            DH_UNROLL for (int i = 0; i < 3; ++i) {
                y[i] = Rj[i * 3] * x[0] + Rj[i * 3 + 1] * x[1] + Rj[i * 3 + 2] * x[2] + T_all[j * 3 + i];
                g[i] = Rj[i * 3] * rays_d[b * 3] + Rj[i * 3 + 1] * rays_d[b * 3 + 1] + Rj[i * 3 + 2] * rays_d[b * 3 + 2];
            }
            if (y[2] > 1e-3f) {
                const float iz = 1.f / y[2];
                const float eu = fx * y[0] * iz + cx - corr[b * 4 + 0], ev = fy * y[1] * iz + cy - corr[b * 4 + 1];
                const float e2 = eu * eu + ev * ev;
                const float en = sqrtf(e2 + 1e-24f);
                const float sres = en / fx;
                res = en;
                const float rho = sres <= delta ? sres * sres / (2.f * delta) : sres - 0.5f * delta;
                const float dpu = fx * (g[0] * y[2] - y[0] * g[2]) * iz * iz, dpv = fy * (g[1] * y[2] - y[1] * g[2]) * iz * iz;
                const float ep = eu * dpu + ev * dpv;
                const float drho = sres <= delta ? ep / (fx * fx * delta) : ep / (en * fx);
                a_cv += conf; a_l += conf * rho; a_r += conf * en;
                dt = conf * drho;
                if (pose_adj) {
                    const float kappa = conf * (sres <= delta ? 1.f / (fx * fx * delta) : 1.f / (en * fx));
                    dy[0] = kappa * eu * fx * iz;
                    dy[1] = kappa * ev * fy * iz;
                    dy[2] = -kappa * (eu * fx * y[0] + ev * fy * y[1]) * iz * iz;
                    DH_UNROLL for (int c = 0; c < 3; ++c) dx[c] = Rj[c] * dy[0] + Rj[3 + c] * dy[1] + Rj[6 + c] * dy[2];
                }
            }
            depth_out = depth;
        }
        residual_px[b] = res;
        d_weights[b * n] = dt;
        if (pose_adj) {
            float* pa = pose_adj + b * 7;
            pa[0] = dx[0]; pa[1] = dx[1]; pa[2] = dx[2]; pa[3] = dy[0]; pa[4] = dy[1]; pa[5] = dy[2]; pa[6] = depth_out;
        }
    }
    const float cv = block_sum(a_cv, s_red), ls = block_sum(a_l, s_red), rs = block_sum(a_r, s_red);
    const float inv = corr_w / (cv + 1e-5f);
    __syncthreads();
    __shared__ float s_dt[1024];
    for (int64_t b0 = 0; b0 < B; b0 += blockDim.x) {
        const int64_t b = b0 + tid;
        s_dt[tid] = b < B ? d_weights[b * n] * inv : 0.f;
        __syncthreads();
        const int64_t nb = (B - b0) < (int64_t)blockDim.x ? (B - b0) : (int64_t)blockDim.x;
        for (int64_t e = tid; e < nb * n; e += blockDim.x) {
            const int64_t r = e / n; const int k = (int)(e % n);
            const float* zr = z + (b0 + r) * n;
            const float dist = (k + 1 < n) ? zr[k + 1] - zr[k] : sample_dist;
            d_weights[(b0 + r) * n + k] = s_dt[r] * (zr[k] + 0.5f * dist);
        }
        __syncthreads();
    }
    if (pose_adj)
        for (int64_t e = tid; e < B * 7; e += blockDim.x) if (e % 7 != 6) pose_adj[e] *= inv;
    if (tid == 0) {
        stats[0] = ls / (cv + 1e-5f);
        stats[1] = cv;
        stats[2] = rs / (cv + 1e-5f);
        stats[3] = corr_w * stats[0];
    }
}

int launch_loss(const float* color, const float* wsum, const float* nmap, const float* eik, const float* rays,
                const float* R, int64_t B, float igr_w, float mask_w, float normal_w, float* stats, float* d_color,
                float* d_wsum, float* d_nmap, float* eik_coef, hipStream_t st) {
    hipLaunchKernelGGL(loss_kernel, dim3(1), dim3(1024), 0, st, color, wsum, nmap, eik, rays, R, B, igr_w, mask_w, normal_w,
                       stats, d_color, d_wsum, d_nmap, eik_coef);
    return hipGetLastError() == hipSuccess ? 0 : -3;
}

int launch_corr_loss(const float* rays_o, const float* rays_d, const float* z, const float* weights, const float* corr,
                     const float* R_all, const float* T_all, int n_frames, const float* K, int64_t B, int n, float sample_dist,
                     float delta_px, float corr_w, float* stats, float* residual_px, float* d_weights, float* pose_adj,
                     hipStream_t st) {
    hipLaunchKernelGGL(corr_loss_kernel, dim3(1), dim3(1024), 0, st, rays_o, rays_d, z, weights, corr, R_all, T_all, n_frames, K, B, n,
                       sample_dist, delta_px, corr_w, stats, residual_px, d_weights, pose_adj);
    return hipGetLastError() == hipSuccess ? 0 : -3;
}

int launch_adam(float* p, const float* g, float* m, float* v, int64_t n, float lr, float b1, float b2, float eps,
                int64_t step, float grad_scale, hipStream_t st) {
    const double bc1 = 1.0 - pow((double)b1, (double)step);
    const double bc2 = 1.0 - pow((double)b2, (double)step);
    hipLaunchKernelGGL(adam_kernel, dim3((unsigned)((n + 255) / 256)), dim3(256), 0, st, p, g, m, v, n, lr, b1, b2, eps,
                       (float)bc1, (float)sqrt(bc2), grad_scale);
    return hipGetLastError() == hipSuccess ? 0 : -3;
}

}
```

### dynhor_amd/csrc/pack.hip

```cpp
#include "tile16h.h"
#include "kernels.h"

namespace dh {

__global__ __launch_bounds__(256) void rowscale_kernel(const float* __restrict__ params, float* __restrict__ packed) {
    const int wave = threadIdx.x >> 6, lane = threadIdx.x & 63;
    const int job = blockIdx.y;
    const bool is_sdf = job < N_SDF;
    const int l = is_sdf ? job : job - N_SDF;
    int out, in;
    int64_t goff, voff;
    if (is_sdf) { out = SDF_DIMS[l].out; in = SDF_DIMS[l].in; goff = sdf_off(l).g; voff = sdf_off(l).v; }
    else        { out = COL_DIMS[l].out; in = COL_DIMS[l].in; goff = col_off(l).g; voff = col_off(l).v; }
    __shared__ float wmax[4];
    float rmax = 0.f;
    for (int rr = 0; rr < 4; ++rr) {
        const int row = (blockIdx.x * 4 + rr) * 4 + wave;
        if (row >= out) break;
        const float* v = params + voff + (int64_t)row * in;
        float s = 0.f, vmax = 0.f;
        for (int k = lane; k < in; k += 64) { s += v[k] * v[k]; vmax = fmaxf(vmax, fabsf(v[k])); }
        for (int off = 32; off > 0; off >>= 1) { s += __shfl_xor(s, off); vmax = fmaxf(vmax, __shfl_xor(vmax, off)); }
        const float inv = 1.f / sqrtf(s);
        const float gi = params[goff + row] * inv;
        if (lane == 0) {
            const int64_t ro = PACK.rowscale + (is_sdf ? (int64_t)l * 260 : (int64_t)N_SDF * 260 + (int64_t)l * 256);
            packed[ro + row] = gi;
            packed[ro + row + (PACK.invnorm - PACK.rowscale)] = inv;
        }
        rmax = fmaxf(rmax, fabsf(gi) * vmax);
    }
    if (lane == 0) wmax[wave] = rmax;
    __syncthreads();
    if (threadIdx.x == 0) {
        const float m = fmaxf(fmaxf(wmax[0], wmax[1]), fmaxf(wmax[2], wmax[3]));
        if (m > 0.f) atomicMax(reinterpret_cast<unsigned*>(packed + PACKH.wabs) + job, __builtin_bit_cast(unsigned, m));
    }
}

struct PackJob {
    int64_t dst;
    int64_t voff;
    int64_t rsoff;
    int ldv;
    int nkg;
    int nt;
    int rev;
    int row_off;
    int col_off;
    int out_valid;
    int in_valid;
    float scale;
    int li;
};

struct PackJobs { PackJob j[44]; int n; };

__global__ __launch_bounds__(256) void pack_kernel(const float* __restrict__ params, float* __restrict__ packed, PackJobs jobs) {
    const PackJob J = jobs.j[blockIdx.y];
    const int64_t total4 = (int64_t)J.nkg * J.nt * 64;
    for (int64_t i = blockIdx.x * 256 + threadIdx.x; i < total4; i += (int64_t)gridDim.x * 256) {
        const int lane = i & 63;
        const int nt = (i >> 6) % J.nt;
        const int kg = (i >> 6) / J.nt;
        const int n = nt * 32 + (lane & 31);
        f32x4 v;
        DH_UNROLL for (int s = 0; s < 4; ++s) {
            const int k = kg * 8 + 4 * (lane >> 5) + s;
            const int o = J.rev ? k : n, c = J.rev ? n : k;
            float x = 0.f;
            if (o < J.out_valid && c < J.in_valid) {
                const int row = o + J.row_off;
                x = J.scale * packed[J.rsoff + row] * params[J.voff + (int64_t)row * J.ldv + J.col_off + c];
            }
            v[s] = x;
        }
        reinterpret_cast<f32x4*>(packed + J.dst)[i] = v;
    }
}

__global__ __launch_bounds__(256) void pack_small_kernel(const float* __restrict__ params, float* __restrict__ packed) {
    const int c = threadIdx.x;
    const int job = blockIdx.x;
    if (job < N_SDF) {
        const int l = job;
        float b = 0.f;
        if (l < 8) { if (c < SDF_DIMS[l].out) b = params[sdf_off(l).bias + c]; }
        else b = params[sdf_off(8).bias + 1 + c];
        packed[PACK.sdf_bias[l] + c] = b;
    } else if (job == N_SDF) {
        const int64_t rs = PACK.rowscale + 8 * 260;
        packed[PACK.sdf_w8row0 + c] = packed[rs + 0] * params[sdf_off(8).v + c];
        if (c == 0) packed[PACK.sdf_b8_0] = params[sdf_off(8).bias];
    } else if (job < N_SDF + 1 + 4) {
        const int l = job - N_SDF - 1;
        packed[PACK.col_bias[l] + c] = params[col_off(l).bias + c];
    } else {
        const int64_t rs = PACK.rowscale + (int64_t)N_SDF * 260 + 4 * 256;
        for (int r = 0; r < 3; ++r) packed[PACK.col_w4 + r * 256 + c] = packed[rs + r] * params[col_off(4).v + r * 256 + c];
        if (c < 3) packed[PACK.col_b4 + c] = params[col_off(4).bias + c];
    }
}

__global__ __launch_bounds__(256) void pack16_kernel(const float* __restrict__ params, float* __restrict__ packed, PackJobs jobs) {
    const PackJob J = jobs.j[blockIdx.y];
    const int64_t total = (int64_t)J.nkg * J.nt * 64;
    bf16x8* dst = reinterpret_cast<bf16x8*>(packed + J.dst);
    for (int64_t i = blockIdx.x * 256 + threadIdx.x; i < total; i += (int64_t)gridDim.x * 256) {
        const int lane = i & 63;
        const int nt = (i >> 6) % J.nt;
        const int kc = (i >> 6) / J.nt;
        const int n = nt * 32 + (lane & 31);
        Bf3 w;
        DH_UNROLL for (int s = 0; s < 8; ++s) {
            const int k = kc * 16 + (J.rev == 2 ? 8 * (s >> 2) + 4 * (lane >> 5) + (s & 3) : 8 * (lane >> 5) + s);
            const int o = J.rev == 1 ? k : n, c = J.rev == 1 ? n : k;
            float x = 0.f;
            if (o < J.out_valid && c < J.in_valid) {
                const int row = o + J.row_off;
                x = J.scale * packed[J.rsoff + row] * params[J.voff + (int64_t)row * J.ldv + J.col_off + c];
            }
            __bf16 h1, h2, h3;
            split_f32(x, h1, h2, h3);
            w.p[0][s] = h1; w.p[1][s] = h2; w.p[2][s] = h3;
        }
        DH_UNROLL for (int p = 0; p < 3; ++p) dst[(((int64_t)kc * J.nt + nt) * 3 + p) * 64 + lane] = w.p[p];
    }
}

__global__ __launch_bounds__(256) void packh_kernel(const float* __restrict__ params, float* __restrict__ packed, PackJobs jobs) {
    const PackJob J = jobs.j[blockIdx.y];
    const int64_t total = (int64_t)J.nkg * J.nt * 64;
    u32x4* dst = reinterpret_cast<u32x4*>(packed + J.dst);
    const float sw = wscale_from_bits(reinterpret_cast<const unsigned*>(packed + PACKH.wabs)[J.li]);
    for (int64_t i = blockIdx.x * 256 + threadIdx.x; i < total; i += (int64_t)gridDim.x * 256) {
        const int lane = i & 63;
        const int nt = (i >> 6) % J.nt;
        const int kc = (i >> 6) / J.nt;
        const int n = nt * 32 + (lane & 31);
        float x[8];
        DH_UNROLL for (int s = 0; s < 8; ++s) {
            const int k = kc * 16 + (J.rev == 2 ? 8 * (s >> 2) + 4 * (lane >> 5) + (s & 3) : 8 * (lane >> 5) + s);
            const int o = J.rev == 1 ? k : n, c = J.rev == 1 ? n : k;
            x[s] = 0.f;
            if (o < J.out_valid && c < J.in_valid) {
                const int row = o + J.row_off;
                x[s] = sw * (J.scale * packed[J.rsoff + row] * params[J.voff + (int64_t)row * J.ldv + J.col_off + c]);
            }
        }
        const H2 w = split2(f32x4{x[0], x[1], x[2], x[3]}, f32x4{x[4], x[5], x[6], x[7]});
        DH_UNROLL for (int p = 0; p < 2; ++p) dst[(((int64_t)kc * J.nt + nt) * 2 + p) * 64 + lane] = w.p[p];
    }
}

__global__ __launch_bounds__(256) void packt_small_kernel(const float* __restrict__ params, float* __restrict__ packed) {
    const int c = threadIdx.x, l = blockIdx.x;
    float v;
    if (l < 8) v = c < SDF_DIMS[l].out ? params[sdf_off(l).bias + c] : 0.f;
    else if (l == 8) v = packed[PACK.rowscale + 8 * 260] * params[sdf_off(8).v + c];
    else v = params[sdf_off(8).bias + 1 + c];
    packed[PACKT.bias10 + l * 256 + c] = v;
}

__global__ __launch_bounds__(256) void packth_small_kernel(const float* __restrict__ params, float* __restrict__ packed) {
    const int c = threadIdx.x, l = blockIdx.x;
    float v;
    if (l < 8) v = c < SDF_DIMS[l].out ? H2_XS * params[sdf_off(l).bias + c] : 0.f;
    else if (l == 8) v = packed[PACK.rowscale + 8 * 260] * params[sdf_off(8).v + c];
    else if (l == 9) v = params[sdf_off(8).bias + 1 + c];
    else v = c < N_SDF ? winv_from_bits(reinterpret_cast<const unsigned*>(packed + PACKH.wabs)[c]) : 0.f;
    packed[PACKH.bias11 + l * 256 + c] = v;
}

template <class OFF>
static PackJobs build_jobs_split(const OFF& P, int64_t ts, int NP) {
    PackJobs J{};
    int n = 0;
    auto add = [&](int64_t dst, int64_t voff, int64_t rsoff, int ldv, int nkc, int nt, int rev, int row_off, int col_off,
                   int out_valid, int in_valid, float scale, int li) {
        J.j[n++] = PackJob{dst, voff, rsoff, ldv, nkc, nt, rev, row_off, col_off, out_valid, in_valid, scale, li};
    };
    for (int l = 0; l < N_SDF; ++l) {
        const int64_t rs = PACK.rowscale + (int64_t)l * 260;
        const int64_t v = sdf_off(l).v;
        const int in = SDF_DIMS[l].in, out = SDF_DIMS[l].out;
        if (l == 0) {
            add(P.sdf_fwd_aux[0], v, rs, in, 3, 8, 0, 0, 0, out, EMB, 1.f, l);
            add(P.sdf_rev_aux[0], v, rs, in, 16, 2, 1, 0, 0, out, EMB, 1.f, l);
        } else if (l == 4) {
            add(P.sdf_fwd_main[4], v, rs, in, 14, 8, 0, 0, 0, out, SKIP_OUT, INV_SQRT2, l);
            add(P.sdf_fwd_aux[4], v, rs, in, 3, 8, 0, 0, SKIP_OUT, out, EMB, INV_SQRT2, l);
            add(P.sdf_rev_main[4], v, rs, in, 16, 8, 1, 0, 0, out, SKIP_OUT, INV_SQRT2, l);
            add(P.sdf_rev_aux[4], v, rs, in, 16, 2, 1, 0, SKIP_OUT, out, EMB, INV_SQRT2, l);
        } else if (l == 8) {
            add(P.sdf_fwd_main[8], v, rs, in, 16, 8, 0, 1, 0, 256, 256, 1.f, l);
            add(P.sdf_rev_main[8], v, rs, in, 16, 8, 1, 1, 0, 256, 256, 1.f, l);
        } else {
            add(P.sdf_fwd_main[l], v, rs, in, 16, 8, 0, 0, 0, out, in, 1.f, l);
            add(P.sdf_rev_main[l], v, rs, in, 16, 8, 1, 0, 0, out, in, 1.f, l);
        }
    }
    auto addt = [&](int l, int nstage, int col_off, int in_valid, float scale, int row_off = 0) {
        add(ts, sdf_off(l).v, PACK.rowscale + (int64_t)l * 260, SDF_DIMS[l].in, nstage, 8, 2, row_off, col_off, SDF_DIMS[l].out - row_off, in_valid, scale, l);
        ts += (int64_t)nstage * 8 * NP * 64 * 4;
    };
    addt(0, 3, 0, EMB, 1.f);
    for (int l = 1; l <= 3; ++l) addt(l, 16, 0, 256, 1.f);
    addt(4, 14, 0, SKIP_OUT, INV_SQRT2);
    addt(4, 3, SKIP_OUT, EMB, INV_SQRT2);
    for (int l = 5; l <= 7; ++l) addt(l, 16, 0, 256, 1.f);
    addt(8, 16, 0, 256, 1.f, 1);
    for (int l = 0; l < 4; ++l) {
        const int64_t rs = PACK.rowscale + (int64_t)N_SDF * 260 + (int64_t)l * 256;
        const int64_t v = col_off(l).v;
        const int in = COL_DIMS[l].in;
        if (l == 0) {
            add(P.col_fwd_main[0], v, rs, in, 16, 8, 0, 0, CAUX, 256, 256, 1.f, N_SDF + l);
            add(P.col_fwd_aux0, v, rs, in, 3, 8, 0, 0, 0, 256, CAUX, 1.f, N_SDF + l);
            add(P.col_rev_main[0], v, rs, in, 16, 8, 1, 0, CAUX, 256, 256, 1.f, N_SDF + l);
            add(P.col_rev_aux0, v, rs, in, 16, 2, 1, 0, 0, 256, CAUX, 1.f, N_SDF + l);
        } else {
            add(P.col_fwd_main[l], v, rs, in, 16, 8, 0, 0, 0, 256, 256, 1.f, N_SDF + l);
            add(P.col_rev_main[l], v, rs, in, 16, 8, 1, 0, 0, 256, 256, 1.f, N_SDF + l);
        }
    }
    J.n = n;
    return J;
}

static PackJobs build_jobs() {
    PackJobs J{};
    int n = 0;
    auto add = [&](int64_t dst, int64_t voff, int64_t rsoff, int ldv, int nkg, int nt, int rev, int row_off, int col_off,
                   int out_valid, int in_valid, float scale) {
        J.j[n++] = PackJob{dst, voff, rsoff, ldv, nkg, nt, rev, row_off, col_off, out_valid, in_valid, scale, 0};
    };
    for (int l = 0; l < N_SDF; ++l) {
        const int64_t rs = PACK.rowscale + (int64_t)l * 260;
        const int64_t v = sdf_off(l).v;
        const int in = SDF_DIMS[l].in, out = SDF_DIMS[l].out;
        if (l == 0) {
            add(PACK.sdf_fwd_aux[0], v, rs, in, 5, 8, 0, 0, 0, out, EMB, 1.f);
            add(PACK.sdf_rev_aux[0], v, rs, in, 32, 2, 1, 0, 0, out, EMB, 1.f);
        } else if (l == 4) {
            add(PACK.sdf_fwd_main[4], v, rs, in, 28, 8, 0, 0, 0, out, SKIP_OUT, INV_SQRT2);
            add(PACK.sdf_fwd_aux[4], v, rs, in, 5, 8, 0, 0, SKIP_OUT, out, EMB, INV_SQRT2);
            add(PACK.sdf_rev_main[4], v, rs, in, 32, 8, 1, 0, 0, out, SKIP_OUT, INV_SQRT2);
            add(PACK.sdf_rev_aux[4], v, rs, in, 32, 2, 1, 0, SKIP_OUT, out, EMB, INV_SQRT2);
        } else if (l == 8) {
            add(PACK.sdf_fwd_main[8], v, rs, in, 32, 8, 0, 1, 0, 256, 256, 1.f);
            add(PACK.sdf_rev_main[8], v, rs, in, 32, 8, 1, 1, 0, 256, 256, 1.f);
        } else {
            add(PACK.sdf_fwd_main[l], v, rs, in, 32, 8, 0, 0, 0, out, in, 1.f);
            add(PACK.sdf_rev_main[l], v, rs, in, 32, 8, 1, 0, 0, out, in, 1.f);
        }
    }
    for (int l = 0; l < 4; ++l) {
        const int64_t rs = PACK.rowscale + (int64_t)N_SDF * 260 + (int64_t)l * 256;
        const int64_t v = col_off(l).v;
        const int in = COL_DIMS[l].in;
        if (l == 0) {
            add(PACK.col_fwd_main[0], v, rs, in, 32, 8, 0, 0, CAUX, 256, 256, 1.f);
            add(PACK.col_fwd_aux0, v, rs, in, 5, 8, 0, 0, 0, 256, CAUX, 1.f);
            add(PACK.col_rev_main[0], v, rs, in, 32, 8, 1, 0, CAUX, 256, 256, 1.f);
            add(PACK.col_rev_aux0, v, rs, in, 32, 2, 1, 0, 0, 256, CAUX, 1.f);
        } else {
            add(PACK.col_fwd_main[l], v, rs, in, 32, 8, 0, 0, 0, 256, 256, 1.f);
            add(PACK.col_rev_main[l], v, rs, in, 32, 8, 1, 0, 0, 256, 256, 1.f);
        }
    }
    J.n = n;
    return J;
}

int launch_pack_weights(const float* params, float* packed, int arith_mask, hipStream_t stream) {
    (void)hipMemsetAsync(packed + PACKH.wabs, 0, 16 * sizeof(unsigned), stream);
    hipLaunchKernelGGL(rowscale_kernel, dim3(17, N_SDF + N_COL), dim3(256), 0, stream, params, packed);
    hipLaunchKernelGGL(pack_small_kernel, dim3(N_SDF + 1 + 4 + 1), dim3(256), 0, stream, params, packed);
    if (arith_mask & (1 << ARITH_FP32)) {
        static const PackJobs jobs = build_jobs();
        hipLaunchKernelGGL(pack_kernel, dim3(16, jobs.n), dim3(256), 0, stream, params, packed, jobs);
    }
    if (arith_mask & (1 << ARITH_BF16)) {
        static const PackJobs jobs16 = build_jobs_split(PACK16, PACKT.stream, 3);
        hipLaunchKernelGGL(pack16_kernel, dim3(8, jobs16.n), dim3(256), 0, stream, params, packed, jobs16);
        hipLaunchKernelGGL(packt_small_kernel, dim3(10), dim3(256), 0, stream, params, packed);
    }
    if (arith_mask & (1 << ARITH_F16)) {
        static const PackJobs jobsh = build_jobs_split(PACKH, PACKH.stream, 2);
        hipLaunchKernelGGL(packh_kernel, dim3(8, jobsh.n), dim3(256), 0, stream, params, packed, jobsh);
        hipLaunchKernelGGL(packth_small_kernel, dim3(11), dim3(256), 0, stream, params, packed);
    }
    return hipGetLastError() == hipSuccess ? 0 : -3;
}

}
```

### dynhor_amd/fields.py

```python
from __future__ import annotations


import numpy as np
import torch
import torch.nn as nn

from . import _lib


class _WNLinearParams(nn.Module):

    def __init__(self, weight: torch.Tensor, bias: torch.Tensor):
        super().__init__()
        self.bias = nn.Parameter(bias.clone())
        self.weight_g = nn.Parameter(weight.norm(dim=1, keepdim=True).clone())
        self.weight_v = nn.Parameter(weight.clone())

    def forward(self, *a, **k):
        raise RuntimeError("dynhor_amd modules have no eager forward; use NeuSRenderer (HIP path)")


class SDFNetwork(nn.Module):

    def __init__(self, d_in=3, d_out=257, d_hidden=256, n_layers=8, skip_in=(4,), multires=6, bias=0.5, scale=1.0,
# ... 45 lines not shown
        dims = [d0] + [d_hidden] * n_layers + [d_out]
        self.num_layers = len(dims)
        for l in range(self.num_layers - 1):
            lin = nn.Linear(dims[l], dims[l + 1])
            setattr(self, "lin" + str(l), _WNLinearParams(lin.weight.data, lin.bias.data))


class SingleVarianceNetwork(nn.Module):
    def __init__(self, init_val=0.3):
        super().__init__()
        self.register_parameter("variance", nn.Parameter(torch.tensor(float(init_val))))


class ParamStore:

    def __init__(self, sdf_network: SDFNetwork, deviation_network: SingleVarianceNetwork, color_network: RenderingNetwork,
                 device):
        _lib.lib()
        self.device = torch.device(device)
        self.modules = (sdf_network, deviation_network, color_network)
        self.n, self.slices, self.var_off, packed_floats = self._layout(sdf_network, deviation_network, color_network)
        self.flat = torch.empty(self.n, device=self.device, dtype=torch.float32)
        self.slices.sort(key=lambda s: s[1])
        end = 0
        for p, off, n in self.slices:
            assert off == end, "flat layout must be dense"
            end = off + n
            self.flat[off:off + n].copy_(p.detach().reshape(-1).to(self.device, torch.float32))
            p.data = self.flat[off:off + n].view(p.shape)
        assert end == self.n
        self.packed = torch.empty(packed_floats, device=self.device, dtype=torch.float32)
        self._packed_version = None
        self.grad_flat = None
        self._grad_bucket = None
        self.exp_avg = torch.zeros_like(self.flat)
        self.exp_avg_sq = torch.zeros_like(self.flat)
        self.step_count = 0
        self._manual_version = 0

    def _layout(self, sdf_network, deviation_network, color_network):
        L = _lib.lib()
        slices = []
        for net, mod in ((0, sdf_network), (2, color_network)):
            n_layers = 9 if net == 0 else 5
            for l in range(n_layers):
                b, g, v, out_dim, in_dim = _lib.param_layout(net, l)
                lin = getattr(mod, "lin" + str(l))
                assert tuple(lin.weight_v.shape) == (out_dim, in_dim), (net, l, lin.weight_v.shape)
                slices += [(lin.bias, b, out_dim), (lin.weight_g, g, out_dim), (lin.weight_v, v, out_dim * in_dim)]
        _, _, voff, _, _ = _lib.param_layout(1, 0)
        slices.append((deviation_network.variance, voff, 1))
        return int(L.dh_num_params()), slices, voff, int(L.dh_packed_floats())

    def _pack(self, arithmetic=None):
        if arithmetic is None:
            _lib.check(_lib.lib().dh_pack_weights(_lib.ptr(self.flat), _lib.ptr(self.packed), _lib.stream()))
        else:
            _lib.check(_lib.lib().dh_pack_weights_ex(int(arithmetic), _lib.ptr(self.flat), _lib.ptr(self.packed), _lib.stream()))

    def params(self):
        return [p for p, _, _ in self.slices]

    def grad_bucket(self) -> torch.Tensor:
        if self._grad_bucket is None:
            self._grad_bucket = torch.empty(self.n, device=self.device, dtype=torch.float32)
        return self._grad_bucket

    def bump(self):
        self._manual_version += 1

    def ensure_packed(self, arithmetic=None):
        ver = (self.flat._version, self._manual_version, sum(p._version for p, _, _ in self.slices))
        if ver != self._packed_version:
            self._packed_version = ver
            self._packed_sets = set()
        want = "all" if arithmetic is None else int(arithmetic)
        have = getattr(self, "_packed_sets", set())
        if "all" not in have and want not in have:
            self._pack(arithmetic)
            have.add(want)
            self._packed_sets = have
        return self.packed

    def inv_s(self) -> torch.Tensor:
        return torch.exp(self.flat[self.var_off:self.var_off + 1] * 10.0).clip(1e-6, 1e6)

    def adam_step(self, lr: float, betas=(0.9, 0.999), eps=1e-8, grad: torch.Tensor | None = None, grad_scale=1.0):
        g = grad if grad is not None else self.grad_flat
        if g is None:
            raise RuntimeError("adam_step: no gradient (call backward() first)")
        self.step_count += 1
        _lib.check(_lib.lib().dh_adam_step(_lib.ptr(self.flat), _lib.ptr(g), _lib.ptr(self.exp_avg),
                                           _lib.ptr(self.exp_avg_sq), self.n, float(lr), float(betas[0]), float(betas[1]),
                                           float(eps), self.step_count, float(grad_scale), _lib.stream()))
        self.bump()

    def zero_grad(self):
        for p, _, _ in self.slices:
            p.grad = None
        self.grad_flat = None

    def optimizer_state_dict(self, lr: float, betas=(0.9, 0.999), eps=1e-8):
        state = {}
        for i, (p, off, cnt) in enumerate(self.slices):
            state[i] = {"step": torch.tensor(float(self.step_count)),
                        "exp_avg": self.exp_avg[off:off + cnt].view(p.shape).clone(),
                        "exp_avg_sq": self.exp_avg_sq[off:off + cnt].view(p.shape).clone()}
        group = {"lr": lr, "betas": tuple(betas), "eps": eps, "weight_decay": 0, "amsgrad": False,
                 "maximize": False, "foreach": None, "capturable": False, "differentiable": False, "fused": None,
                 "params": list(range(len(self.slices)))}
        return {"state": state if self.step_count > 0 else {}, "param_groups": [group]}

    def load_optimizer_state_dict(self, sd):
        st = sd.get("state", {})
        if not st:
            self.exp_avg.zero_(); self.exp_avg_sq.zero_(); self.step_count = 0
            return
        for i, (p, off, cnt) in enumerate(self.slices):
            s = st[i] if i in st else st[str(i)]
            self.exp_avg[off:off + cnt].copy_(s["exp_avg"].reshape(-1))
            self.exp_avg_sq[off:off + cnt].copy_(s["exp_avg_sq"].reshape(-1))
            self.step_count = int(float(s["step"]))
```

### dynhor_amd/renderer.py

```python
from __future__ import annotations

import ctypes
from types import SimpleNamespace

import torch

from . import _lib
from .fields import ParamStore, RenderingNetwork, SDFNetwork, SingleVarianceNetwork

_NULL = ctypes.c_void_p(0)


def _p(t):
    return _NULL if t is None else _lib.ptr(t)


class StageTimer:

    def __init__(self):
        self.enabled = False
        self.records = {}
        self.markers = False
        self._roctx = None

# ... 113 lines not shown
          _p(s.colors), save, _lib.stream())

    def _net_backward(self, s, d_sdf, d_normals, d_colors, grad):
        L, T, st = _lib.lib(), self.timer, self.store
        P = s.B * s.n
        ar = s.arith
        if getattr(s, "ray_grads", False):
            s.d_pts = torch.empty(P, 3, device=s.pts.device)
            s.d_dirs_pts = torch.empty(P, 3, device=s.pts.device)
            T("color_backward", L.dh_color_backward_rays_ex, ar, _p(st.packed), _p(s.colors), _p(d_colors), _p(s.rays_d), s.n, P, _p(s.ws),
              _p(d_normals), _p(s.d_pts), _p(s.d_dirs_pts), _lib.stream())
            T("sdf_tangent", L.dh_sdf_tangent_ex, ar, _p(st.packed), _p(s.pts), _p(d_normals), P, _p(s.ws), _lib.stream())
            T("sdf_backward", L.dh_sdf_backward_rays_ex, ar, _p(st.packed), _p(d_sdf), _p(s.pts), _p(d_normals), P, _p(s.ws), _p(s.d_pts),
              _lib.stream())
        else:
            T("color_backward", L.dh_color_backward_ex, ar, _p(st.packed), _p(s.colors), _p(d_colors), P, _p(s.ws), _p(d_normals),
              _lib.stream())
            T("sdf_tangent", L.dh_sdf_tangent_ex, ar, _p(st.packed), _p(s.pts), _p(d_normals), P, _p(s.ws), _lib.stream())
            T("sdf_backward", L.dh_sdf_backward_ex, ar, _p(st.packed), _p(d_sdf), P, _p(s.ws), _lib.stream())
        T("weight_grads_gemm", L.dh_weight_grads_gemm_ex, ar, P, _p(s.ws), _lib.stream())
        T("weight_grads_fold", L.dh_weight_grads_fold, _p(st.packed), _p(st.flat), P, _p(s.ws), _p(grad), _lib.stream())

    def range_status(self, state=None):
        s = state if state is not None else getattr(self, "last_state", None)
        if s is None or getattr(s, "arith", None) != _lib.ARITH_SPLIT_F16:
            return None
        a, _, lim = _lib.range_words()
        return float(s.ws[a]), lim

    def check_range(self, state=None, max_over_ranks=None):
        st = self.range_status(state)
        if st is None:
            if max_over_ranks is not None:
                max_over_ranks(0.0)
            return None
        m, lim = st
        g = max_over_ranks(m) if max_over_ranks is not None else m
        if not g < lim:
            where = "" if g == m or max_over_ranks is None else f" (this rank: {m:.4g}; the maximum is another rank's)"
            raise _lib.DynhorHipError(
                f"split_f16 range exceeded: max softplus activation of the SDF network = {g:.4g}{where}, limit {lim:.0f} (fp16 overflow at "
                "the forward chain's constant scale 16): this step's results are not valid; use model.arithmetic = 'split_bf16'")
        return m, lim

    def sdf(self, pts: torch.Tensor) -> torch.Tensor:
        pts = pts.contiguous().float()
        out = torch.empty(pts.shape[0], device=pts.device)
        self.store.ensure_packed(self._arith())
        self._net_sdf_nograd("sdf_nograd", pts, pts.shape[0], out)
        return out.view(-1, 1)

    @torch.no_grad()
    def extract_geometry(self, bound_min, bound_max, resolution, threshold=0.0, method="cubes", mode="dense", block=8, lipschitz=None):
        from .mesh import marching_cubes, marching_tetrahedra
        if method not in ("cubes", "tetrahedra"):
            raise ValueError("extract_geometry: method must be 'cubes' or 'tetrahedra'")
        if mode not in ("dense", "sparse"):
            raise ValueError("extract_geometry: mode must be 'dense' or 'sparse'")
        if mode == "sparse" and method != "cubes":
            raise ValueError("extract_geometry: mode 'sparse' triangulates by marching cubes only (method 'cubes')")
        dev = self.store.device
        if mode == "sparse":
            from . import mesh_extract
            verts, faces, self.last_extract_stats = mesh_extract.sparse_marching_cubes(
                lambda p: -self.sdf(p), resolution, bound_min, bound_max, threshold=threshold, block=block,
                lipschitz=mesh_extract.DEFAULT_LIPSCHITZ if lipschitz is None else lipschitz, device=dev)
            return verts, faces
        N = int(resolution)
        ax = [torch.linspace(float(bound_min[i]), float(bound_max[i]), N, device=dev) for i in range(3)]
        u = torch.empty(N, N, N, device=dev)
        step = 64
        for xi in range(0, N, step):
            for yi in range(0, N, step):
                for zi in range(0, N, step):
                    gx, gy, gz = torch.meshgrid(ax[0][xi:xi + step], ax[1][yi:yi + step], ax[2][zi:zi + step], indexing="ij")
                    pts = torch.stack([gx, gy, gz], dim=-1).reshape(-1, 3).contiguous()
                    u[xi:xi + step, yi:yi + step, zi:zi + step] = -self.sdf(pts).reshape(gx.shape)
        if not bool(torch.isfinite(u).all()):
            raise _lib.DynhorHipError("extract_geometry: non-finite SDF values on the grid (split_f16 range exceeded, or the network "
                                      "has diverged); use arithmetic 'split_bf16' for queries this far out")
        return (marching_cubes if method == "cubes" else marching_tetrahedra)(u, threshold, bound_min, bound_max)

    @torch.no_grad()
    def sample_z(self, rays_o, rays_d, near, far, perturb_overwrite=-1, t_rand=None):
        L = _lib.lib()
        packed = self.store.ensure_packed(self._arith())
        dev = rays_o.device
        B = rays_o.shape[0]
        ns = self.n_samples
        perturb = self.perturb if perturb_overwrite < 0 else perturb_overwrite
        if perturb > 0 and t_rand is None:
            t_rand = torch.rand([B, 1], device=dev)
        if perturb <= 0:
            t_rand = None
        near = near.contiguous().view(-1)
        far = far.contiguous().view(-1)
        z = torch.empty(B, ns, device=dev)
        pts = torch.empty(B * ns, 3, device=dev)
        _lib.check(L.dh_coarse_samples(_p(rays_o), _p(rays_d), _p(near), _p(far),
                                       _p(t_rand.contiguous().view(-1)) if t_rand is not None else _NULL,
                                       B, ns, _p(z), _p(pts), _lib.stream()))
        if self.n_importance > 0:
            sdf = torch.empty(B * ns, device=dev)
            self._net_sdf_nograd("sdf_nograd_coarse", pts, B * ns, sdf)
            n_new = self.n_importance // self.up_sample_steps
            n_cur = ns
            for i in range(self.up_sample_steps):
                last = (i + 1 == self.up_sample_steps)
                z_new = torch.empty(B, n_new, device=dev)
                pts_new = torch.empty(B * n_new, 3, device=dev)
                _lib.check(L.dh_upsample_step(_p(rays_o), _p(rays_d), _p(z), _p(sdf), B, n_cur, n_new,
                                              float(64 * 2 ** i), _p(z_new), _p(pts_new), _lib.stream()))
                z_out = torch.empty(B, n_cur + n_new, device=dev)
                if not last:
                    sdf_new = torch.empty(B * n_new, device=dev)
                    self._net_sdf_nograd("sdf_nograd_fine", pts_new, B * n_new, sdf_new)
                    sdf_out = torch.empty(B * (n_cur + n_new), device=dev)
                    _lib.check(L.dh_merge_samples(_p(z), _p(z_new), _p(sdf), _p(sdf_new), B, n_cur, n_new, _p(z_out),
                                                  _p(sdf_out), _lib.stream()))
                    sdf = sdf_out
                else:
                    _lib.check(L.dh_merge_samples(_p(z), _p(z_new), _NULL, _NULL, B, n_cur, n_new, _p(z_out), _NULL,
                                                  _lib.stream()))
                z = z_out
                n_cur += n_new
        return z

    @torch.no_grad()
    def _forward_core(self, rays_o, rays_d, z_vals, cos_anneal_ratio, background_rgb, want_nmap, infer_only=False,
                      ray_grads=False):
        L = _lib.lib()
        st = self.store
        packed = st.ensure_packed(self._arith())
        dev = rays_o.device
        B, n = z_vals.shape
        P = B * n
        s = SimpleNamespace()
        s.B, s.n, s.car, s.sample_dist = B, n, float(cos_anneal_ratio), 2.0 / self.n_samples
        s.rays_o, s.rays_d, s.z_vals, s.bg = rays_o, rays_d, z_vals, background_rgb
        s.ws = self._workspace(P, infer_only)
        s.infer_only = infer_only
        s.ray_grads = bool(ray_grads) and not infer_only
        self._ws_token += 1
        s.ws_token = self._ws_token
        s.pts = torch.empty(P, 3, device=dev)
        s.sdf = torch.empty(P, device=dev)
        s.normals = torch.empty(P, 3, device=dev)
        s.colors = torch.empty(P, 3, device=dev)
        _lib.check(L.dh_midpoints(_p(rays_o), _p(rays_d), _p(z_vals), B, n, s.sample_dist, _p(s.pts), _lib.stream()))
        self._net_forward(s, packed)
        s.inv_s = st.inv_s()
        s.weights = torch.empty(B, n, device=dev)
        s.color = torch.empty(B, 3, device=dev)
        s.wsum = torch.empty(B, 1, device=dev)
        s.wmax = torch.empty(B, 1, device=dev)
        s.cdf = torch.empty(B, n, device=dev)
        s.inside = torch.empty(B, n, device=dev)
        s.eik = torch.empty(B, 2, device=dev)
        s.nmap = torch.empty(B, 3, device=dev) if want_nmap else None
        _lib.check(L.dh_render_scan_fwd(_p(rays_o), _p(rays_d), _p(z_vals), _p(s.sdf), _p(s.normals), _p(s.colors),
                                        _p(s.inv_s), s.car, s.sample_dist, _p(background_rgb), B, n, _p(s.weights),
                                        _p(s.color), _p(s.wsum), _p(s.wmax), _p(s.cdf), _p(s.inside), _p(s.eik),
                                        _p(s.nmap), _lib.stream()))
        return s

    @torch.no_grad()
    def _backward_core(self, s, d_color, d_wsum, d_weights, d_gradients, d_nmap, eik_coef, d_sdf_out=None, persistent=False):
        L = _lib.lib()
        st = self.store
        if s.infer_only:
            raise RuntimeError("this forward pass was run with infer_only=True: nothing was saved for backward")
        if s.ws_token != self._ws_token:
            raise RuntimeError("NeuSRenderer workspace was overwritten by a later render() call before backward(); "
                               "call backward() before rendering again (one live graph per renderer)")
        B, n = s.B, s.n
        P = B * n
        dev = s.color.device
        c = lambda t: None if t is None else t.contiguous()
        d_color = c(d_color) if d_color is not None else torch.zeros(B, 3, device=dev)
        d_sdf = torch.empty(P, device=dev)
        d_normals = torch.empty(P, 3, device=dev)
        d_colors = torch.empty(P, 3, device=dev)
        d_inv_s = torch.empty(B, device=dev)
        if s.ray_grads:
            d_rays_d = torch.empty(B, 3, device=dev)
            _lib.check(L.dh_render_scan_bwd_rays(_p(s.rays_o), _p(s.rays_d), _p(s.z_vals), _p(s.sdf), _p(s.normals), _p(s.colors),
                                                 _p(s.inv_s), s.car, s.sample_dist, _p(s.bg), B, n, _p(d_color), _p(c(d_wsum)),
                                                 _p(c(d_weights)), _p(c(d_gradients)), _p(c(d_nmap)), _p(eik_coef), _p(d_sdf),
                                                 _p(d_normals), _p(d_colors), _p(d_inv_s), _p(d_rays_d), _lib.stream()))
        else:
            _lib.check(L.dh_render_scan_bwd(_p(s.rays_o), _p(s.rays_d), _p(s.z_vals), _p(s.sdf), _p(s.normals), _p(s.colors),
                                            _p(s.inv_s), s.car, s.sample_dist, _p(s.bg), B, n, _p(d_color), _p(c(d_wsum)),
                                            _p(c(d_weights)), _p(c(d_gradients)), _p(c(d_nmap)), _p(eik_coef), _p(d_sdf),
                                            _p(d_normals), _p(d_colors), _p(d_inv_s), _lib.stream()))
        if d_sdf_out is not None:
            d_sdf = (d_sdf + d_sdf_out.reshape(-1)).contiguous()
        grad = st.grad_bucket() if persistent else torch.empty(st.n, device=dev)
        self._net_backward(s, d_sdf, d_normals, d_colors, grad)
        raw = torch.exp(st.flat[st.var_off] * 10.0)
        passthrough = ((raw >= 1e-6) & (raw <= 1e6)).float()
        grad[st.var_off] = d_inv_s.sum() * 10.0 * raw * passthrough
        st.grad_flat = grad
        if s.ray_grads:
            dz = torch.cat([s.z_vals[:, 1:] - s.z_vals[:, :-1], torch.full_like(s.z_vals[:, :1], s.sample_dist)], -1)
            mid = (s.z_vals + 0.5 * dz).unsqueeze(-1)
            dp = s.d_pts.view(B, n, 3)
            s.d_rays_o = dp.sum(dim=1)
            s.d_rays_d = (dp * mid).sum(dim=1) + s.d_dirs_pts.view(B, n, 3).sum(dim=1) + d_rays_d
        return grad

    @torch.no_grad()
    def render_rays(self, rays_o, rays_d, near, far, cos_anneal_ratio, background_rgb=None, want_nmap=True):
        z = self.sample_z(rays_o, rays_d, near, far, perturb_overwrite=0)
        st = self._forward_core(rays_o, rays_d, z, cos_anneal_ratio, background_rgb, want_nmap=want_nmap, infer_only=True)
        return st.color, st.nmap

    def render(self, rays_o, rays_d, near, far, perturb_overwrite=-1, background_rgb=None, cos_anneal_ratio=0.0,
               t_rand=None, z_vals=None):
        if rays_o.dim() != 2 or rays_o.shape[1] != 3 or rays_d.shape != rays_o.shape:
            raise ValueError("rays_o / rays_d must be [B,3]")
        if rays_o.dtype != torch.float32 or not rays_o.is_cuda:
            raise TypeError("rays must be fp32 tensors on the HIP device")
        rays_o = rays_o.contiguous()
        rays_d = rays_d.contiguous()
        B = rays_o.shape[0]
        if z_vals is None:
            z_vals = self.sample_z(rays_o, rays_d, near, far, perturb_overwrite, t_rand)
        z_vals = z_vals.contiguous()
        bg = None if background_rgb is None else background_rgb.reshape(-1).contiguous().float()
        outs = _RenderCoreFn.apply(self, rays_o, rays_d, z_vals, cos_anneal_ratio, bg, *self.store.params())
        color, wsum, gradient_error, weights, gradients, wmax, cdf, inside, sdf = outs
        inv_s = self.store.inv_s()
        s_val = (1.0 / inv_s).expand(B, 1)
        return {
            "color_fine": color, "s_val": s_val, "cdf_fine": cdf, "weight_sum": wsum, "weight_max": wmax,
            "gradients": gradients, "weights": weights, "gradient_error": gradient_error, "inside_sphere": inside,
            "z_vals": z_vals, "sdf": sdf,
        }

    @torch.no_grad()
    def train_step_core(self, rays, near, far, R, cos_anneal_ratio, igr_weight=0.1, mask_weight=0.1, normal_weight=0.0,
                        background_rgb=None, t_rand=None, corr=None, corr_weight=0.0, corr_frames=None, corr_delta_px=4.0,
                        ray_grads=False):
        L = _lib.lib()
        dev = rays.device
        B = rays.shape[0]
        rays_o = rays[:, 0:3].contiguous()
        rays_d = rays[:, 3:6].contiguous()
        z_vals = self.sample_z(rays_o, rays_d, near, far, t_rand=t_rand)
        bg = None if background_rgb is None else background_rgb.reshape(-1).contiguous().float()
        s = self._forward_core(rays_o, rays_d, z_vals, cos_anneal_ratio, bg, want_nmap=normal_weight > 0.0, ray_grads=ray_grads)
        stats = torch.empty(8, device=dev)
        d_color = torch.empty(B, 3, device=dev)
        d_wsum = torch.empty(B, device=dev)
        d_nmap = torch.empty(B, 3, device=dev) if normal_weight > 0.0 else None
        eik_coef = torch.empty(1, device=dev)
        Rc = R.contiguous().float() if R is not None else None
        _lib.check(L.dh_neus_loss(_p(s.color), _p(s.wsum), _p(s.nmap), _p(s.eik), _p(rays), _p(Rc), B, float(igr_weight),
                                  float(mask_weight), float(normal_weight), _p(stats), _p(d_color), _p(d_wsum),
                                  _p(d_nmap), _p(eik_coef), _lib.stream()))
        d_weights = None
        if corr is not None and corr_weight > 0.0:
            R_all, T_all, K = corr_frames
            cstats = torch.empty(4, device=dev)
            resid = torch.empty(B, device=dev)
            d_weights = torch.empty(B, s.n, device=dev)
            pose_adj = torch.empty(B, 7, device=dev) if ray_grads else None
            _lib.check(L.dh_corr_loss(_p(rays_o), _p(rays_d), _p(z_vals), _p(s.weights), _p(corr.contiguous()),
                                      _p(R_all.contiguous()), _p(T_all.contiguous()), int(R_all.shape[0]), _p(K.contiguous()),
                                      B, s.n, s.sample_dist, float(corr_delta_px), float(corr_weight), _p(cstats), _p(resid),
                                      _p(d_weights), _p(pose_adj), _lib.stream()))
            stats[0] += cstats[3]
            self.last_corr_stats, self.last_corr_residual_px = cstats, resid
        self._backward_core(s, d_color, d_wsum, d_weights, None, d_nmap, eik_coef, persistent=True)
        self.last_state = s
        if ray_grads:
            d_R = None
            if normal_weight > 0.0 and Rc is not None:
                d_R = (d_nmap @ Rc.T).T @ s.nmap
            self.last_partner_pose_grads = None
            if corr is not None and corr_weight > 0.0:
                d_x, d_y, t_hat = pose_adj[:, 0:3], pose_adj[:, 3:6], pose_adj[:, 6:7]
                s.d_rays_o = s.d_rays_o + d_x
                s.d_rays_d = s.d_rays_d + t_hat * d_x
                x = rays_o + t_hat * rays_d
                j = corr[:, 3].long().clamp(0, R_all.shape[0] - 1)
                d_R_all = torch.zeros_like(R_all).index_add_(0, j, d_y[:, :, None] * x[:, None, :])
                d_T_all = torch.zeros_like(T_all).index_add_(0, j, d_y)
                self.last_partner_pose_grads = (d_R_all, d_T_all)
            self.last_ray_grads = (s.d_rays_o, s.d_rays_d, d_R)
        return stats
```

### include/dynhor_hip.h

```cpp
#ifndef DYNHOR_HIP_H
#define DYNHOR_HIP_H
#include <stddef.h>
#include <stdint.h>

#ifdef __cplusplus
extern "C" {
#endif

typedef enum {
    DH_OK = 0,
    DH_ERR_BAD_ARG = -1,
    DH_ERR_UNSUPPORTED = -2,
    DH_ERR_LAUNCH = -3
} dh_status;

int dh_version(void);
const char* dh_strerror(int status);

typedef enum { DH_ARITH_SPLIT_BF16 = 0, DH_ARITH_FP32_MFMA = 1, DH_ARITH_SPLIT_F16 = 2 } dh_arithmetic;
enum { DH_CHAIN_FORM_TILE = 0x100, DH_CHAIN_FORM_PAIR = 0x200 };
int dh_set_arithmetic(int mode);
int dh_get_arithmetic(void);

int64_t dh_num_params(void);
int64_t dh_packed_floats(void);
int dh_param_layout(int net, int layer, int64_t* bias_off, int64_t* g_off, int64_t* v_off, int* out_dim, int* in_dim);

int dh_packed_section(int section, int64_t* offset_floats, int64_t* n_floats);

int dh_pack_weights(const float* params, float* packed, void* stream);

int dh_sdf_nograd(const float* packed, const float* pts, int64_t npts, float* sdf, void* stream);

int dh_workspace_floats(int64_t npts, int64_t* infer_floats, int64_t* fwd_floats, int64_t* total_floats);

int dh_range_words(int64_t* act_max_off, int64_t* tag_off, float* limit);

int dh_mlp_forward(const float* packed, const float* pts, const float* dirs, int n_per_ray, int64_t npts, float* ws,
                   float* sdf, float* normals, float* color, void* stream);

int dh_sdf_forward(const float* packed, const float* pts, int64_t npts, float* ws, float* sdf, void* stream);
int dh_sdf_gradient(const float* packed, const float* pts, int64_t npts, float* ws, float* normals, int save, void* stream);
int dh_color_forward(const float* packed, const float* pts, const float* dirs, int n_per_ray, const float* normals,
                     int64_t npts, float* ws, float* color, int save, void* stream);

int dh_mlp_backward(const float* packed, const float* params, const float* pts, int64_t npts, float* ws,
                    const float* colors, const float* d_sdf, float* d_normals, const float* d_colors, float* grad_flat,
                    void* stream);

int dh_color_backward(const float* packed, const float* colors, const float* d_colors, int64_t npts, float* ws,
                      float* d_normals, void* stream);
int dh_sdf_tangent(const float* packed, const float* pts, const float* d_normals, int64_t npts, float* ws, void* stream);
int dh_sdf_backward(const float* packed, const float* d_sdf, int64_t npts, float* ws, void* stream);
int dh_color_backward_rays(const float* packed, const float* colors, const float* d_colors, const float* dirs, int n_per_ray,
                           int64_t npts, float* ws, float* d_normals, float* d_pts, float* d_dirs_pts, void* stream);
int dh_sdf_backward_rays(const float* packed, const float* d_sdf, const float* pts, const float* d_normals, int64_t npts,
                         float* ws, float* d_pts, void* stream);
int dh_weight_grads_gemm(int64_t npts, float* ws, void* stream);
int dh_weight_grads_fold(const float* packed, const float* params, int64_t npts, float* ws, float* grad_flat, void* stream);

int dh_sdf_nograd_ex(int arithmetic, const float* packed, const float* pts, int64_t npts, float* sdf, void* stream);
int dh_mlp_forward_ex(int arithmetic, const float* packed, const float* pts, const float* dirs, int n_per_ray, int64_t npts, float* ws,
                      float* sdf, float* normals, float* color, void* stream);
int dh_sdf_forward_ex(int arithmetic, const float* packed, const float* pts, int64_t npts, float* ws, float* sdf, void* stream);
int dh_sdf_gradient_ex(int arithmetic, const float* packed, const float* pts, int64_t npts, float* ws, float* normals, int save,
                       void* stream);
int dh_color_forward_ex(int arithmetic, const float* packed, const float* pts, const float* dirs, int n_per_ray, const float* normals,
                        int64_t npts, float* ws, float* color, int save, void* stream);
int dh_mlp_backward_ex(int arithmetic, const float* packed, const float* params, const float* pts, int64_t npts, float* ws,
                       const float* colors, const float* d_sdf, float* d_normals, const float* d_colors, float* grad_flat,
                       void* stream);
int dh_color_backward_ex(int arithmetic, const float* packed, const float* colors, const float* d_colors, int64_t npts, float* ws,
                         float* d_normals, void* stream);
int dh_sdf_tangent_ex(int arithmetic, const float* packed, const float* pts, const float* d_normals, int64_t npts, float* ws,
                      void* stream);
int dh_sdf_backward_ex(int arithmetic, const float* packed, const float* d_sdf, int64_t npts, float* ws, void* stream);
int dh_color_backward_rays_ex(int arithmetic, const float* packed, const float* colors, const float* d_colors, const float* dirs,
                              int n_per_ray, int64_t npts, float* ws, float* d_normals, float* d_pts, float* d_dirs_pts, void* stream);
int dh_sdf_backward_rays_ex(int arithmetic, const float* packed, const float* d_sdf, const float* pts, const float* d_normals,
                            int64_t npts, float* ws, float* d_pts, void* stream);
int dh_weight_grads_gemm_ex(int arithmetic, int64_t npts, float* ws, void* stream);
int dh_pack_weights_ex(int arithmetic, const float* params, float* packed, void* stream);

int dh_gen_rays(const uint8_t* rgb, const int8_t* label, const uint8_t* normal, const float* R, const float* T,
                const float* Kinv, int H, int W, int n_frames, int frame, const int64_t* px, const int64_t* py, int64_t B,
                float* rays, float* near, float* far, void* stream);

int dh_coarse_samples(const float* rays_o, const float* rays_d, const float* near, const float* far, const float* t_rand,
                      int64_t B, int n_samples, float* z, float* pts, void* stream);

int dh_upsample_step(const float* rays_o, const float* rays_d, const float* z, const float* sdf, int64_t B, int n_cur,
                     int n_new, float inv_s, float* z_new, float* pts_new, void* stream);

int dh_merge_samples(const float* z, const float* z_new, const float* sdf, const float* sdf_new, int64_t B, int n_cur,
                     int n_new, float* z_out, float* sdf_out, void* stream);

int dh_midpoints(const float* rays_o, const float* rays_d, const float* z, int64_t B, int n, float sample_dist, float* pts,
                 void* stream);

int dh_render_scan_fwd(const float* rays_o, const float* rays_d, const float* z, const float* sdf, const float* normals,
                       const float* colors, const float* inv_s, float cos_anneal_ratio, float sample_dist,
                       const float* background_rgb, int64_t B, int n, float* weights, float* color, float* weight_sum,
                       float* weight_max, float* cdf, float* inside_sphere, float* eik_partial, float* normal_map,
                       void* stream);

int dh_render_scan_bwd(const float* rays_o, const float* rays_d, const float* z, const float* sdf, const float* normals,
                       const float* colors, const float* inv_s, float cos_anneal_ratio, float sample_dist,
                       const float* background_rgb, int64_t B, int n, const float* d_color, const float* d_weight_sum,
                       const float* d_weights, const float* d_gradients, const float* d_normal_map, const float* eik_coef,
                       float* d_sdf, float* d_normals, float* d_colors, float* d_inv_s, void* stream);
int dh_render_scan_bwd_rays(const float* rays_o, const float* rays_d, const float* z, const float* sdf, const float* normals,
                            const float* colors, const float* inv_s, float cos_anneal_ratio, float sample_dist,
                            const float* background_rgb, int64_t B, int n, const float* d_color, const float* d_weight_sum,
                            const float* d_weights, const float* d_gradients, const float* d_normal_map, const float* eik_coef,
                            float* d_sdf, float* d_normals, float* d_colors, float* d_inv_s, float* d_rays_d, void* stream);

int dh_neus_loss(const float* color, const float* weight_sum, const float* normal_map, const float* eik_partial,
                 const float* rays, const float* R, int64_t B, float igr_weight, float mask_weight, float normal_weight,
                 float* stats, float* d_color, float* d_weight_sum, float* d_normal_map, float* eik_coef, void* stream);

int dh_corr_loss(const float* rays_o, const float* rays_d, const float* z, const float* weights, const float* corr,
                 const float* R_all, const float* T_all, int n_frames, const float* K, int64_t B, int n, float sample_dist,
                 float delta_px, float corr_weight, float* stats, float* residual_px, float* d_weights, float* pose_adjoints,
                 void* stream);

int dh_march_count(const float* rays_o, const float* rays_d, const float* near, const float* far, const float* u,
                   const uint8_t* occupancy, int res, float radius, float step, float half_step, int max_samples, int64_t B,
                   int32_t* cnt, void* stream);
int dh_march_emit(const float* rays_o, const float* rays_d, const float* near, const float* far, const float* u,
                  const uint8_t* occupancy, int res, float radius, float step, float half_step, int max_samples, int64_t B,
                  const int64_t* off, const int32_t* keep, float* t_start, float* pts, float* dirs_pts, int32_t* ray_idx,
                  void* stream);
int dh_render_scan_fwd_packed(const float* rays_o, const float* rays_d, const float* t_start, const float* sdf, const float* normals,
                              const float* colors, const float* inv_s, float cos_anneal_ratio, float step,
                              const float* background_rgb, int64_t B, const int64_t* seg_off, const int32_t* seg_cnt,
                              float* weights, float* color, float* weight_sum, float* weight_max, float* cdf,
                              float* inside_sphere, float* eik_partial, float* normal_map, void* stream);
int dh_render_scan_bwd_packed(const float* rays_o, const float* rays_d, const float* t_start, const float* sdf, const float* normals,
                              const float* colors, const float* inv_s, float cos_anneal_ratio, float step,
                              const float* background_rgb, int64_t B, const int64_t* seg_off, const int32_t* seg_cnt,
                              const float* d_color, const float* d_weight_sum, const float* d_weights, const float* d_gradients,
                              const float* d_normal_map, const float* eik_coef, float* d_sdf, float* d_normals, float* d_colors,
                              float* d_inv_s, void* stream);

int dh_adam_step(float* params, const float* grad, float* exp_avg, float* exp_avg_sq, int64_t n, float lr, float beta1,
                 float beta2, float eps, int64_t step, float grad_scale, void* stream);

int64_t dh_hashgrid_entries(void);
int dh_hashgrid_level(int level, float* scale, uint32_t* resolution, uint32_t* offset, uint32_t* dense);
int dh_hashgrid_encode(const float* table, const float* x01, int64_t n, float* out, void* stream);
int dh_hashgrid_encode_backward(const float* x01, const float* d_out, int64_t n, float* d_table, void* stream);

int64_t dh_hash_num_params(void);
int64_t dh_hash_packed_floats(void);
int dh_hash_param_layout(int net, int layer, int64_t* bias_off, int64_t* g_off, int64_t* v_off, int* out_dim, int* in_dim);
int dh_hash_pack_weights(const float* params, float* packed, void* stream);
int dh_hash_workspace_floats(int64_t npts, int64_t* infer_floats, int64_t* total_floats);
int dh_hash_sdf_nograd(const float* params, const float* packed, const float* pts, int64_t n, float radius, float* sdf,
                       void* stream);
int dh_hash_geo_forward(const float* params, const float* packed, const float* pts, int64_t n, float radius, float eps,
                        float* ws, int save, float* sdf, float* feature, float* gradient, const int64_t* n_active, void* stream);
int dh_hash_color_forward(const float* packed, const float* feature, const float* normals, const float* dirs,
                          int n_per_ray, int64_t n, float* color, const int64_t* n_active, void* stream);
int dh_hash_color_backward(const float* packed, const float* feature, const float* normals, const float* dirs,
                           const float* d_color, int n_per_ray, int64_t n, float* ws, float* d_feature, float* d_normals,
                           const int64_t* n_active, void* stream);
int dh_hash_geo_backward(const float* params, const float* packed, const float* pts, const float* d_sdf,
                         const float* d_feature, const float* d_normals, int64_t n, float radius, float eps, float* ws,
                         const int64_t* n_active, void* stream);
int dh_hash_weight_grads(const float* params, const float* packed, int64_t n, float* ws, float* grad, const int64_t* n_active,
                         void* stream);
int dh_hash_weight_grads_parts(const float* params, const float* packed, int64_t n, float* ws, float* grad, const int64_t* n_active,
                               int parts, void* stream);
int dh_hash_set_scatter_mode(int mode);

int64_t dh_nearest_sqdist_workspace(int64_t nq, int64_t nr);
int dh_nearest_sqdist(const float* q, int64_t nq, const float* ref, int64_t nr, float* d2, int32_t* idx, void* ws, void* stream);

int dh_mesh_sdf_record_floats(void);
int dh_mesh_sdf_prepare(const float* verts, int64_t nv, const int32_t* faces, int64_t nf, float* rec, void* stream);
int64_t dh_mesh_sdf_query_workspace(int64_t n, int64_t nf);
int dh_mesh_sdf_query(const float* rec, int64_t nf, const float* pts, int64_t n, float* sqdist, int32_t* face, float* wind, void* ws,
                      void* stream);

int64_t dh_icp_correspond_workspace(int64_t n, int64_t m, int64_t h);
int dh_icp_correspond(const float* src, int64_t n, const float* tgt, int64_t m, const float* xf, int64_t h, float* d2, int32_t* idx,
                      void* ws, void* stream);
int dh_icp_moments_sums(int plane);
int64_t dh_icp_moments_workspace(int64_t n, int64_t h, int plane);
int dh_icp_moments(const float* src, const float* tgt, const float* tgt_normals, const float* xf, const int32_t* idx, const float* d2,
                   const float* thr, const float* origin_src, const float* origin_tgt, int64_t n, int64_t m, int64_t h, double* out,
                   void* ws, void* stream);

int dh_label_dilate(const int8_t* label, int64_t n_frames, int H, int W, int radius, uint8_t* tmp, uint8_t* keep, void* stream);
int dh_mesh_mask_votes(const float* verts, int64_t nv, const uint8_t* keep, const float* R, const float* T, const float* K,
                       int64_t n_frames, int H, int W, int32_t* bg_votes, int32_t* seen, void* stream);
int dh_mesh_components(const int64_t* faces, int64_t nf, int64_t nv, int32_t* labels, void* stream);

int dh_hull_accumulate(const float* pts, int64_t n, const float* sd, const float* R, const float* T, const float* K, int64_t n_frames,
                       int H, int W, int frame0, int m, float* topk, int32_t* arg, int32_t* seen, void* stream);

int dh_mesh_raster_depth(const float* verts, int64_t nv, const int64_t* faces, int64_t nf, const float* R, const float* T,
                         const float* K, int64_t n_frames, int H, int W, uint64_t* zbuf, void* stream);
int dh_mesh_bake_colors(const float* verts, const float* normals, int64_t nv, const uint8_t* rgb, const uint8_t* usable,
                        const uint64_t* zbuf, const float* R, const float* T, const float* K, int64_t n_frames, int H, int W,
                        float depth_eps, float min_cos, float* acc, int32_t* n_views, void* stream);

int dh_mesh_shade(const float* verts, const float* normals, const uint8_t* colors, int64_t nv, const int64_t* faces, int64_t nf,
                  const uint64_t* zbuf, const float* R, const float* T, const float* K, int64_t n_frames, int H, int W,
                  const uint8_t* rgb, const int8_t* label, float alpha, uint8_t* out, int64_t* counts, void* stream);

int dh_texture_bake(const float* verts, const float* normals, int64_t nv, const int64_t* faces, int64_t nf, const float* uv,
                    const int32_t* owner, int S, const uint8_t* rgb, const uint8_t* usable, const uint64_t* zbuf, const float* R,
                    const float* T, const float* K, int64_t n_frames, int H, int W, float depth_eps, float min_cos, int sharpen,
                    float* acc, int32_t* n_views, void* stream);
int dh_mesh_shade_tex(const float* verts, const float* normals, int64_t nv, const int64_t* faces, int64_t nf, const float* uv,
                      const uint8_t* tex, int Sh, int Sw, const uint64_t* zbuf, const float* R, const float* T, const float* K,
                      int64_t n_frames, int H, int W, const uint8_t* rgb, const uint8_t* usable, float alpha, int lit, uint8_t* out,
                      int64_t* sums, void* stream);

int dh_label_edt(const int8_t* label, int64_t n_frames, int H, int W, int value, int rmax, float* tmp, float* out, void* stream);
int64_t dh_sil_nearest_workspace(int64_t n_frames, int H, int W);
int dh_sil_nearest(const float* verts, int64_t nv, const int64_t* faces, int64_t nf, const float* R, const float* T, const float* K,
                   int64_t n_frames, int H, int W, float rmax_px, uint64_t* near, void* ws, void* stream);
int dh_sil_loss_sums(void);
int64_t dh_sil_loss_grad_workspace(int64_t n_frames, int H, int W);
int dh_sil_loss_grad(const uint64_t* near, const float* verts, int64_t nv, const int64_t* faces, int64_t nf, const float* R,
                     const float* T, const float* K, const float* d2_obj, const float* d2_hand, const int8_t* label, int64_t n_frames,
                     int H, int W, float sigma, float cut, float edge_offset, double* out, void* ws, void* stream);

// ... 61 lines not shown
```

Baseline: 230,300 rays/s.

## Fuse merge with next upsample step and sample tail, add variance-grad kernel

Merges each hierarchical sample-merge with the following upsample step in a single per-ray wave kernel, and fuses the final upsample, merge and midpoint computation into one tail kernel that passes points straight to the forward core. It also replaces the small torch ops for the inv_s variance gradient with a dedicated kernel. The aim is fewer kernel launches and fewer global round trips in the sampling stage, at the cost of more complex kernels with extra LDS use.

```diff
diff --git a/dynhor_amd/_lib.py b/dynhor_amd/_lib.py
--- a/dynhor_amd/_lib.py
+++ b/dynhor_amd/_lib.py
@@ -73,6 +73,9 @@
     "dh_upsample_step": (_i32, [_vp] * 4 + [_i64, _i32, _i32, _f32, _vp, _vp, _vp]),
     "dh_merge_samples": (_i32, [_vp] * 4 + [_i64, _i32, _i32, _vp, _vp, _vp]),
     "dh_midpoints": (_i32, [_vp] * 3 + [_i64, _i32, _f32, _vp, _vp]),
+    "dh_merge_upsample_step": (_i32, [_vp] * 6 + [_i64, _i32, _i32, _i32, _f32] + [_vp] * 5),
+    "dh_sample_tail": (_i32, [_vp] * 6 + [_i64, _i32, _i32, _i32, _f32, _f32, _vp, _vp, _vp]),
+    "dh_variance_grad": (_i32, [_vp, _i64, _vp, _vp, _i64, _vp]),
     "dh_render_scan_fwd": (_i32, [_vp] * 7 + [_f32, _f32, _vp, _i64, _i32] + [_vp] * 9),
     "dh_render_scan_bwd": (_i32, [_vp] * 7 + [_f32, _f32, _vp, _i64, _i32] + [_vp] * 11),
     "dh_render_scan_bwd_rays": (_i32, [_vp] * 7 + [_f32, _f32, _vp, _i64, _i32] + [_vp] * 12),
diff --git a/dynhor_amd/csrc/api.hip b/dynhor_amd/csrc/api.hip
--- a/dynhor_amd/csrc/api.hip
+++ b/dynhor_amd/csrc/api.hip
@@ -14,6 +14,7 @@
 
 namespace {
 inline bool misaligned16(const void* p) { return (reinterpret_cast<uintptr_t>(p) & 15u) != 0; }
+inline bool misaligned4(const void* p) { return (reinterpret_cast<uintptr_t>(p) & 3u) != 0; }
 inline bool bad_arith(int a) { return a != DH_ARITH_SPLIT_BF16 && a != DH_ARITH_FP32_MFMA && a != DH_ARITH_SPLIT_F16; }
 inline bool bad_arith_form(int a) {
     const int form = a & ~0xff;
@@ -318,6 +319,32 @@
     return launch_midpoints(rays_o, rays_d, z, B, n, sample_dist, pts, static_cast<hipStream_t>(stream));
 }
 
+int dh_merge_upsample_step(const float* rays_o, const float* rays_d, const float* z, const float* z_new, const float* sdf,
+                           const float* sdf_new, int64_t B, int n_cur, int n_new, int n_next, float inv_s, float* z_out,
+                           float* sdf_out, float* z_next, float* pts_next, void* stream) {
+    if (B < 0 || n_cur <= 0 || n_new <= 0 || n_next <= 0) return DH_ERR_BAD_ARG;
+    if (n_cur + (int64_t)n_new > 128 || n_new > 64 || n_next > 64) return DH_ERR_UNSUPPORTED;
+    if (B == 0) return DH_OK;
+    if (!rays_o || !rays_d || !z || !z_new || !sdf || !sdf_new || !z_out || !sdf_out || !z_next || !pts_next) return DH_ERR_BAD_ARG;
+    if (misaligned4(rays_o) || misaligned4(rays_d) || misaligned4(z) || misaligned4(z_new) || misaligned4(sdf) || misaligned4(sdf_new) ||
+        misaligned4(z_out) || misaligned4(sdf_out) || misaligned4(z_next) || misaligned4(pts_next)) return DH_ERR_BAD_ARG;
+    return launch_merge_upsample(rays_o, rays_d, z, z_new, sdf, sdf_new, B, n_cur, n_new, n_next, inv_s, z_out, sdf_out, z_next,
+                                 pts_next, static_cast<hipStream_t>(stream));
+}
+
+int dh_sample_tail(const float* rays_o, const float* rays_d, const float* z, const float* z_new, const float* sdf,
+                   const float* sdf_new, int64_t B, int n_cur, int n_new, int n_next, float inv_s, float sample_dist,
+                   float* z_vals, float* pts, void* stream) {
+    if (B < 0 || n_cur <= 0 || n_new <= 0 || n_next <= 0) return DH_ERR_BAD_ARG;
+    if (n_cur + (int64_t)n_new + n_next > 128 || n_new > 64 || n_next > 64) return DH_ERR_UNSUPPORTED;
+    if (B == 0) return DH_OK;
+    if (!rays_o || !rays_d || !z || !z_new || !sdf || !sdf_new || !z_vals || !pts) return DH_ERR_BAD_ARG;
+    if (misaligned4(rays_o) || misaligned4(rays_d) || misaligned4(z) || misaligned4(z_new) || misaligned4(sdf) || misaligned4(sdf_new) ||
+        misaligned4(z_vals) || misaligned4(pts)) return DH_ERR_BAD_ARG;
+    return launch_sample_tail(rays_o, rays_d, z, z_new, sdf, sdf_new, B, n_cur, n_new, n_next, inv_s, sample_dist, z_vals, pts,
+                              static_cast<hipStream_t>(stream));
+}
+
 int dh_render_scan_fwd(const float* rays_o, const float* rays_d, const float* z, const float* sdf, const float* normals,
                        const float* colors, const float* inv_s, float cos_anneal_ratio, float sample_dist,
                        const float* background_rgb, int64_t B, int n, float* weights, float* color, float* weight_sum,
@@ -422,6 +449,13 @@
     if (!params || !grad || !exp_avg || !exp_avg_sq) return DH_ERR_BAD_ARG;
     return launch_adam(params, grad, exp_avg, exp_avg_sq, n, lr, beta1, beta2, eps, step, grad_scale,
                        static_cast<hipStream_t>(stream));
+}
+
+int dh_variance_grad(const float* d_inv_s, int64_t B, const float* raw, float* grad, int64_t var_off, void* stream) {
+    if (B < 0 || var_off < 0) return DH_ERR_BAD_ARG;
+    if (!raw || !grad || (B > 0 && !d_inv_s)) return DH_ERR_BAD_ARG;
+    if (misaligned4(d_inv_s) || misaligned4(raw) || misaligned4(grad)) return DH_ERR_BAD_ARG;
+    return launch_variance_grad(d_inv_s, B, raw, grad + var_off, static_cast<hipStream_t>(stream));
 }
 
 int dh_neus_loss(const float* color, const float* weight_sum, const float* normal_map, const float* eik_partial,
diff --git a/dynhor_amd/csrc/kernels.h b/dynhor_amd/csrc/kernels.h
--- a/dynhor_amd/csrc/kernels.h
+++ b/dynhor_amd/csrc/kernels.h
@@ -73,6 +73,12 @@
                  float* z_out, float* sdf_out, hipStream_t st);
 int launch_midpoints(const float* o, const float* d, const float* z, int64_t B, int n, float sample_dist, float* pts,
                      hipStream_t st);
+int launch_merge_upsample(const float* o, const float* d, const float* z, const float* z_new, const float* sdf, const float* sdf_new,
+                          int64_t B, int n, int n_new, int n_next, float inv_s, float* z_out, float* sdf_out, float* z_next,
+                          float* pts_next, hipStream_t st);
+int launch_sample_tail(const float* o, const float* d, const float* z, const float* z_new, const float* sdf, const float* sdf_new,
+                       int64_t B, int n, int n_new, int n_next, float inv_s, float sample_dist, float* z_fin, float* pts_fin,
+                       hipStream_t st);
 int launch_render_fwd(const float* o, const float* d, const float* z, const float* sdf, const float* normals,
                       const float* colors, const float* inv_s, float car, float sample_dist, const float* bg, int64_t B,
                       int n, float* weights, float* color, float* wsum, float* wmax, float* cdf, float* inside, float* eik,
@@ -132,6 +138,7 @@
 
 int launch_adam(float* p, const float* g, float* m, float* v, int64_t n, float lr, float b1, float b2, float eps,
                 int64_t step, float grad_scale, hipStream_t st);
+int launch_variance_grad(const float* d_inv_s, int64_t B, const float* raw, float* grad_var, hipStream_t st);
 
 int64_t hashgrid_entries();
 int hashgrid_level(int l, float* scale, uint32_t* res, uint32_t* offset, uint32_t* dense);
diff --git a/dynhor_amd/csrc/kernels_ray.hip b/dynhor_amd/csrc/kernels_ray.hip
--- a/dynhor_amd/csrc/kernels_ray.hip
+++ b/dynhor_amd/csrc/kernels_ray.hip
@@ -90,22 +90,20 @@
     DH_UNROLL for (int c = 0; c < 3; ++c) pts[i * 3 + c] = rays_o[b * 3 + c] + rays_d[b * 3 + c] * zz;
 }
 
-__global__ __launch_bounds__(256) void upsample_kernel(const float* __restrict__ rays_o, const float* __restrict__ rays_d,
-                                                       const float* __restrict__ z, const float* __restrict__ sdf,
-                                                       int64_t B, int n, int n_new, float inv_s,
-                                                       float* __restrict__ z_new, float* __restrict__ pts_new) {
-    __shared__ float s_cdf[4][132];
-    __shared__ float s_z[4][132];
-    const int wave = threadIdx.x >> 6, lane = threadIdx.x & 63;
-    const int64_t ray = (int64_t)blockIdx.x * 4 + wave;
-    if (ray >= B) return;
-    const float ox = rays_o[ray * 3], oy = rays_o[ray * 3 + 1], oz = rays_o[ray * 3 + 2];
-    const float dx = rays_d[ray * 3], dy = rays_d[ray * 3 + 1], dz = rays_d[ray * 3 + 2];
+struct RayGeom { float ox, oy, oz, dx, dy, dz; };
+__device__ __forceinline__ RayGeom load_ray(const float* __restrict__ rays_o, const float* __restrict__ rays_d, int64_t ray) {
+    return RayGeom{rays_o[ray * 3], rays_o[ray * 3 + 1], rays_o[ray * 3 + 2], rays_d[ray * 3], rays_d[ray * 3 + 1], rays_d[ray * 3 + 2]};
+}
+__device__ __forceinline__ void wave_lds_sync() {
+    __builtin_amdgcn_fence(__ATOMIC_RELEASE, "workgroup");
+    __builtin_amdgcn_wave_barrier();
+    __builtin_amdgcn_fence(__ATOMIC_ACQUIRE, "workgroup");
+}
+
+__device__ __forceinline__ float upsample_ray(const RayGeom& g, float z0, float z1, float f0, float f1, int n, int n_new, float inv_s,
+                                              int lane, float* cdf, float* zs, float* __restrict__ z_new, float* __restrict__ pts_new) {
+    const float ox = g.ox, oy = g.oy, oz = g.oz, dx = g.dx, dy = g.dy, dz = g.dz;
     const int e0 = 2 * lane, e1 = e0 + 1;
-    const float* zr = z + ray * n;
-    const float* sr = sdf + ray * n;
-    const float z0 = e0 < n ? zr[e0] : 0.f, z1 = e1 < n ? zr[e1] : 0.f;
-    const float f0 = e0 < n ? sr[e0] : 0.f, f1 = e1 < n ? sr[e1] : 0.f;
     auto radius = [&](float t) {
         const float x = ox + dx * t, y = oy + dy * t, w = oz + dz * t;
         return sqrtf(x * x + y * y + w * w);
@@ -136,16 +134,13 @@
     const float tot = wave_sum(wA + wB);
     const float pA = wA / tot, pB = wB / tot;
     const float incl = wave_incl_sum(pA + pB, lane);
-    float* cdf = s_cdf[wave];
-    float* zs = s_z[wave];
     if (lane == 0) cdf[0] = 0.f;
     if (vA) cdf[e0 + 1] = incl - pB;
     if (vB) cdf[e1 + 1] = incl;
     if (e0 < n) zs[e0] = z0;
     if (e1 < n) zs[e1] = z1;
-    __builtin_amdgcn_fence(__ATOMIC_RELEASE, "workgroup");
-    __builtin_amdgcn_wave_barrier();
-    __builtin_amdgcn_fence(__ATOMIC_ACQUIRE, "workgroup");
+    wave_lds_sync();
+    float zn = 0.f;
     if (lane < n_new) {
         const float u = (0.5f + (float)lane) / (float)n_new;
         int lo = 0, hi = n;
@@ -159,11 +154,53 @@
         if (denom < 1e-5f) denom = 1.f;
         const float t = (u - c0) / denom;
         const float b0 = zs[below], b1 = zs[above];
-        const float zn = b0 + t * (b1 - b0);
-        z_new[ray * n_new + lane] = zn;
-        float* pp = pts_new + (ray * n_new + lane) * 3;
-        pp[0] = ox + dx * zn; pp[1] = oy + dy * zn; pp[2] = oz + dz * zn;
-    }
+        zn = b0 + t * (b1 - b0);
+        if (z_new) {
+            z_new[lane] = zn;
+            float* pp = pts_new + lane * 3;
+            pp[0] = ox + dx * zn; pp[1] = oy + dy * zn; pp[2] = oz + dz * zn;
+        }
+    }
+    return zn;
+}
+
+__device__ __forceinline__ void merge_ranks(float z0, float z1, float zn, int n_new, int lane, int& c0, int& c1, int& cn) {
+    c0 = 0; c1 = 0; cn = 0;
+    for (int k = 0; k < n_new; ++k) {
+        const float v = __shfl(zn, k);
+        c0 += (v < z0) ? 1 : 0;
+        c1 += (v < z1) ? 1 : 0;
+    }
+    for (int k = 0; k < n_new; ++k) {
+        const float v = __shfl(zn, k);
+        const int cnt = __popcll(__ballot(z0 <= v)) + __popcll(__ballot(z1 <= v));
+        if (lane == k) cn = cnt;
+    }
+}
+
+__device__ __forceinline__ void midpoint_elem(const float (&o)[3], const float (&d)[3], float zc, float znext, bool last,
+                                              float sample_dist, float* __restrict__ p) {
+    const float dist = last ? sample_dist : znext - zc;
+    const float mid = zc + dist * 0.5f;
+    DH_UNROLL for (int c = 0; c < 3; ++c) p[c] = o[c] + d[c] * mid;
+}
+
+__global__ __launch_bounds__(256) void upsample_kernel(const float* __restrict__ rays_o, const float* __restrict__ rays_d,
+                                                       const float* __restrict__ z, const float* __restrict__ sdf,
+                                                       int64_t B, int n, int n_new, float inv_s,
+                                                       float* __restrict__ z_new, float* __restrict__ pts_new) {
+    __shared__ float s_cdf[4][132];
+    __shared__ float s_z[4][132];
+    const int wave = threadIdx.x >> 6, lane = threadIdx.x & 63;
+    const int64_t ray = (int64_t)blockIdx.x * 4 + wave;
+    if (ray >= B) return;
+    const RayGeom g = load_ray(rays_o, rays_d, ray);
+    const int e0 = 2 * lane, e1 = e0 + 1;
+    const float* zr = z + ray * n;
+    const float* sr = sdf + ray * n;
+    const float z0 = e0 < n ? zr[e0] : 0.f, z1 = e1 < n ? zr[e1] : 0.f;
+    const float f0 = e0 < n ? sr[e0] : 0.f, f1 = e1 < n ? sr[e1] : 0.f;
+    upsample_ray(g, z0, z1, f0, f1, n, n_new, inv_s, lane, s_cdf[wave], s_z[wave], z_new + ray * n_new, pts_new + ray * n_new * 3);
 }
 
 __global__ __launch_bounds__(256) void merge_kernel(const float* __restrict__ z, const float* __restrict__ z_new,
@@ -177,17 +214,8 @@
     const float INF = __builtin_inff();
     const float z0 = e0 < n ? z[ray * n + e0] : INF, z1 = e1 < n ? z[ray * n + e1] : INF;
     const float zn = lane < n_new ? z_new[ray * n_new + lane] : INF;
-    int c0 = 0, c1 = 0, cn = 0;
-    for (int k = 0; k < n_new; ++k) {
-        const float v = __shfl(zn, k);
-        c0 += (v < z0) ? 1 : 0;
-        c1 += (v < z1) ? 1 : 0;
-    }
-    for (int k = 0; k < n_new; ++k) {
-        const float v = __shfl(zn, k);
-        const int cnt = __popcll(__ballot(z0 <= v)) + __popcll(__ballot(z1 <= v));
-        if (lane == k) cn = cnt;
-    }
+    int c0, c1, cn;
+    merge_ranks(z0, z1, zn, n_new, lane, c0, c1, cn);
     const int no = n + n_new;
     float* zo = z_out + ray * no;
     if (e0 < n) zo[e0 + c0] = z0;
@@ -208,9 +236,72 @@
     if (i >= B * n) return;
     const int64_t b = i / n;
     const int j = (int)(i - b * n);
-    const float dist = (j + 1 < n) ? z[i + 1] - z[i] : sample_dist;
-    const float mid = z[i] + dist * 0.5f;
-    DH_UNROLL for (int c = 0; c < 3; ++c) pts[i * 3 + c] = rays_o[b * 3 + c] + rays_d[b * 3 + c] * mid;
+    const float o[3] = {rays_o[b * 3], rays_o[b * 3 + 1], rays_o[b * 3 + 2]};
+    const float d[3] = {rays_d[b * 3], rays_d[b * 3 + 1], rays_d[b * 3 + 2]};
+    const bool last = j + 1 >= n;
+    midpoint_elem(o, d, z[i], last ? 0.f : z[i + 1], last, sample_dist, pts + i * 3);
+}
+
+template <bool TAIL>
+__global__ __launch_bounds__(256) void merge_upsample_kernel(const float* __restrict__ rays_o, const float* __restrict__ rays_d,
+                                                             const float* __restrict__ z, const float* __restrict__ z_new,
+                                                             const float* __restrict__ sdf, const float* __restrict__ sdf_new,
+                                                             int64_t B, int n, int n_new, int n_next, float inv_s, float sample_dist,
+                                                             float* __restrict__ z_out, float* __restrict__ sdf_out,
+                                                             float* __restrict__ z_next, float* __restrict__ pts_next,
+                                                             float* __restrict__ z_fin, float* __restrict__ pts_fin) {
+    __shared__ float s_cdf[4][132];
+    __shared__ float s_z[4][132];
+    __shared__ float s_f[4][132];
+    __shared__ float s_o[TAIL ? 4 : 1][132];
+    const int wave = threadIdx.x >> 6, lane = threadIdx.x & 63;
+    const int64_t ray = (int64_t)blockIdx.x * 4 + wave;
+    if (ray >= B) return;
+    const RayGeom g = load_ray(rays_o, rays_d, ray);
+    const int e0 = 2 * lane, e1 = e0 + 1;
+    const float INF = __builtin_inff();
+    float* zs = s_z[wave];
+    float* fs = s_f[wave];
+    const int nm = n + n_new;
+    {
+        const float z0 = e0 < n ? z[ray * n + e0] : INF, z1 = e1 < n ? z[ray * n + e1] : INF;
+        const float zn = lane < n_new ? z_new[ray * n_new + lane] : INF;
+        int c0, c1, cn;
+        merge_ranks(z0, z1, zn, n_new, lane, c0, c1, cn);
+        if (e0 < n) { zs[e0 + c0] = z0; fs[e0 + c0] = sdf[ray * n + e0]; }
+        if (e1 < n) { zs[e1 + c1] = z1; fs[e1 + c1] = sdf[ray * n + e1]; }
+        if (lane < n_new) { zs[lane + cn] = zn; fs[lane + cn] = sdf_new[ray * n_new + lane]; }
+    }
+    wave_lds_sync();
+    const bool v0 = e0 < nm, v1 = e1 < nm;
+    const float m0 = v0 ? zs[e0] : 0.f, m1 = v1 ? zs[e1] : 0.f;
+    const float h0 = v0 ? fs[e0] : 0.f, h1 = v1 ? fs[e1] : 0.f;
+    if (!TAIL) {
+        if (v0) { z_out[ray * nm + e0] = m0; sdf_out[ray * nm + e0] = h0; }
+        if (v1) { z_out[ray * nm + e1] = m1; sdf_out[ray * nm + e1] = h1; }
+    }
+    const float zq = upsample_ray(g, m0, m1, h0, h1, nm, n_next, inv_s, lane, s_cdf[wave], zs,
+                                  TAIL ? nullptr : z_next + ray * n_next, TAIL ? nullptr : pts_next + ray * n_next * 3);
+    if (TAIL) {
+        float* os = s_o[wave];
+        const int nf = nm + n_next;
+        int c0, c1, cn;
+        merge_ranks(v0 ? m0 : INF, v1 ? m1 : INF, lane < n_next ? zq : INF, n_next, lane, c0, c1, cn);
+        if (v0) os[e0 + c0] = m0;
+        if (v1) os[e1 + c1] = m1;
+        if (lane < n_next) os[lane + cn] = zq;
+        wave_lds_sync();
+        const float o[3] = {g.ox, g.oy, g.oz}, d[3] = {g.dx, g.dy, g.dz};
+        DH_UNROLL for (int k = 0; k < 2; ++k) {
+            const int e = e0 + k;
+            if (e < nf) {
+                const bool last = e + 1 >= nf;
+                const float zc = os[e];
+                z_fin[ray * nf + e] = zc;
+                midpoint_elem(o, d, zc, last ? 0.f : os[e + 1], last, sample_dist, pts_fin + (ray * nf + e) * 3);
+            }
+        }
+    }
 }
 
 struct RenderElem {
@@ -440,6 +531,21 @@
     hipLaunchKernelGGL(midpoints_kernel, dim3((unsigned)((B * n + 255) / 256)), dim3(256), 0, st, o, d, z, B, n, sample_dist, pts);
     return ok();
 }
+int launch_merge_upsample(const float* o, const float* d, const float* z, const float* z_new, const float* sdf, const float* sdf_new,
+                          int64_t B, int n, int n_new, int n_next, float inv_s, float* z_out, float* sdf_out, float* z_next,
+                          float* pts_next, hipStream_t st) {
+    hipLaunchKernelGGL(merge_upsample_kernel<false>, dim3((unsigned)((B + 3) / 4)), dim3(256), 0, st, o, d, z, z_new, sdf, sdf_new, B,
+                       n, n_new, n_next, inv_s, 0.f, z_out, sdf_out, z_next, pts_next, (float*)nullptr, (float*)nullptr);
+    return ok();
+}
+int launch_sample_tail(const float* o, const float* d, const float* z, const float* z_new, const float* sdf, const float* sdf_new,
+                       int64_t B, int n, int n_new, int n_next, float inv_s, float sample_dist, float* z_fin, float* pts_fin,
+                       hipStream_t st) {
+    hipLaunchKernelGGL(merge_upsample_kernel<true>, dim3((unsigned)((B + 3) / 4)), dim3(256), 0, st, o, d, z, z_new, sdf, sdf_new, B,
+                       n, n_new, n_next, inv_s, sample_dist, (float*)nullptr, (float*)nullptr, (float*)nullptr, (float*)nullptr,
+                       z_fin, pts_fin);
+    return ok();
+}
 int launch_render_fwd(const float* o, const float* d, const float* z, const float* sdf, const float* normals,
                       const float* colors, const float* inv_s, float car, float sample_dist, const float* bg, int64_t B,
                       int n, float* weights, float* color, float* wsum, float* wmax, float* cdf, float* inside, float* eik,
diff --git a/dynhor_amd/csrc/optim.hip b/dynhor_amd/csrc/optim.hip
--- a/dynhor_amd/csrc/optim.hip
+++ b/dynhor_amd/csrc/optim.hip
@@ -185,6 +185,27 @@
     }
 }
 
+__global__ __launch_bounds__(256) void variance_grad_kernel(const float* __restrict__ d_inv_s, int64_t B, const float* __restrict__ raw_p,
+                                                            float* __restrict__ grad_var) {
+    __shared__ double s_red[4];
+    double a = 0.0;
+    for (int64_t b = threadIdx.x; b < B; b += 256) a += (double)d_inv_s[b];
+    DH_UNROLL for (int off = 32; off > 0; off >>= 1) a += __shfl_xor(a, off);
+    if ((threadIdx.x & 63) == 0) s_red[threadIdx.x >> 6] = a;
+    __syncthreads();
+    if (threadIdx.x == 0) {
+        const float sum = (float)(((s_red[0] + s_red[1]) + s_red[2]) + s_red[3]);
+        const float raw = raw_p[0];
+        const float g = (sum * 10.0f) * raw;
+        grad_var[0] = (raw >= 1e-6f && raw <= 1e6f) ? g : 0.f;
+    }
+}
+
+int launch_variance_grad(const float* d_inv_s, int64_t B, const float* raw, float* grad_var, hipStream_t st) {
+    hipLaunchKernelGGL(variance_grad_kernel, dim3(1), dim3(256), 0, st, d_inv_s, B, raw, grad_var);
+    return hipGetLastError() == hipSuccess ? 0 : -3;
+}
+
 int launch_loss(const float* color, const float* wsum, const float* nmap, const float* eik, const float* rays,
                 const float* R, int64_t B, float igr_w, float mask_w, float normal_w, float* stats, float* d_color,
                 float* d_wsum, float* d_nmap, float* eik_coef, hipStream_t st) {
diff --git a/dynhor_amd/csrc/pack.hip b/dynhor_amd/csrc/pack.hip
--- a/dynhor_amd/csrc/pack.hip
+++ b/dynhor_amd/csrc/pack.hip
@@ -79,9 +79,8 @@
     }
 }
 
-__global__ __launch_bounds__(256) void pack_small_kernel(const float* __restrict__ params, float* __restrict__ packed) {
-    const int c = threadIdx.x;
-    const int job = blockIdx.x;
+constexpr int PACK_SMALL_BLOCKS = N_SDF + 1 + 4 + 1;
+__device__ __forceinline__ void pack_small_block(const float* __restrict__ params, float* __restrict__ packed, int job, int c) {
     if (job < N_SDF) {
         const int l = job;
         float b = 0.f;
@@ -100,6 +99,9 @@
         for (int r = 0; r < 3; ++r) packed[PACK.col_w4 + r * 256 + c] = packed[rs + r] * params[col_off(4).v + r * 256 + c];
         if (c < 3) packed[PACK.col_b4 + c] = params[col_off(4).bias + c];
     }
+}
+__global__ __launch_bounds__(256) void pack_small_kernel(const float* __restrict__ params, float* __restrict__ packed) {
+    pack_small_block(params, packed, blockIdx.x, threadIdx.x);
 }
 
 __global__ __launch_bounds__(256) void pack16_kernel(const float* __restrict__ params, float* __restrict__ packed, PackJobs jobs) {
@@ -128,12 +130,12 @@
     }
 }
 
-__global__ __launch_bounds__(256) void packh_kernel(const float* __restrict__ params, float* __restrict__ packed, PackJobs jobs) {
-    const PackJob J = jobs.j[blockIdx.y];
+constexpr int PACKH_BLOCKS_PER_JOB = 8;
+__device__ __forceinline__ void packh_block(const float* __restrict__ params, float* __restrict__ packed, const PackJob& J, int bx, int nbx) {
     const int64_t total = (int64_t)J.nkg * J.nt * 64;
     u32x4* dst = reinterpret_cast<u32x4*>(packed + J.dst);
     const float sw = wscale_from_bits(reinterpret_cast<const unsigned*>(packed + PACKH.wabs)[J.li]);
-    for (int64_t i = blockIdx.x * 256 + threadIdx.x; i < total; i += (int64_t)gridDim.x * 256) {
+    for (int64_t i = bx * 256 + threadIdx.x; i < total; i += (int64_t)nbx * 256) {
         const int lane = i & 63;
         const int nt = (i >> 6) % J.nt;
         const int kc = (i >> 6) / J.nt;
@@ -152,6 +154,9 @@
         DH_UNROLL for (int p = 0; p < 2; ++p) dst[(((int64_t)kc * J.nt + nt) * 2 + p) * 64 + lane] = w.p[p];
     }
 }
+__global__ __launch_bounds__(256) void packh_kernel(const float* __restrict__ params, float* __restrict__ packed, PackJobs jobs) {
+    packh_block(params, packed, jobs.j[blockIdx.y], blockIdx.x, gridDim.x);
+}
 
 __global__ __launch_bounds__(256) void packt_small_kernel(const float* __restrict__ params, float* __restrict__ packed) {
     const int c = threadIdx.x, l = blockIdx.x;
@@ -162,14 +167,24 @@
     packed[PACKT.bias10 + l * 256 + c] = v;
 }
 
-__global__ __launch_bounds__(256) void packth_small_kernel(const float* __restrict__ params, float* __restrict__ packed) {
-    const int c = threadIdx.x, l = blockIdx.x;
+constexpr int PACKTH_SMALL_BLOCKS = 11;
+__device__ __forceinline__ void packth_small_block(const float* __restrict__ params, float* __restrict__ packed, int l, int c) {
     float v;
     if (l < 8) v = c < SDF_DIMS[l].out ? H2_XS * params[sdf_off(l).bias + c] : 0.f;
     else if (l == 8) v = packed[PACK.rowscale + 8 * 260] * params[sdf_off(8).v + c];
     else if (l == 9) v = params[sdf_off(8).bias + 1 + c];
     else v = c < N_SDF ? winv_from_bits(reinterpret_cast<const unsigned*>(packed + PACKH.wabs)[c]) : 0.f;
     packed[PACKH.bias11 + l * 256 + c] = v;
+}
+__global__ __launch_bounds__(256) void packth_small_kernel(const float* __restrict__ params, float* __restrict__ packed) {
+    packth_small_block(params, packed, blockIdx.x, threadIdx.x);
+}
+
+__global__ __launch_bounds__(256) void pack_f16_kernel(const float* __restrict__ params, float* __restrict__ packed, PackJobs jobs) {
+    const int b = blockIdx.x, nh = PACKH_BLOCKS_PER_JOB * jobs.n;
+    if (b < nh) packh_block(params, packed, jobs.j[b / PACKH_BLOCKS_PER_JOB], b % PACKH_BLOCKS_PER_JOB, PACKH_BLOCKS_PER_JOB);
+    else if (b < nh + PACK_SMALL_BLOCKS) pack_small_block(params, packed, b - nh, threadIdx.x);
+    else packth_small_block(params, packed, b - nh - PACK_SMALL_BLOCKS, threadIdx.x);
 }
 
 template <class OFF>
@@ -276,7 +291,12 @@
 int launch_pack_weights(const float* params, float* packed, int arith_mask, hipStream_t stream) {
     (void)hipMemsetAsync(packed + PACKH.wabs, 0, 16 * sizeof(unsigned), stream);
     hipLaunchKernelGGL(rowscale_kernel, dim3(17, N_SDF + N_COL), dim3(256), 0, stream, params, packed);
-    hipLaunchKernelGGL(pack_small_kernel, dim3(N_SDF + 1 + 4 + 1), dim3(256), 0, stream, params, packed);
+#ifdef DH_PACK_SPLIT
+    const bool fuse_f16 = false;
+#else
+    const bool fuse_f16 = (arith_mask & (1 << ARITH_F16)) != 0;
+#endif
+    if (!fuse_f16) hipLaunchKernelGGL(pack_small_kernel, dim3(PACK_SMALL_BLOCKS), dim3(256), 0, stream, params, packed);
     if (arith_mask & (1 << ARITH_FP32)) {
         static const PackJobs jobs = build_jobs();
         hipLaunchKernelGGL(pack_kernel, dim3(16, jobs.n), dim3(256), 0, stream, params, packed, jobs);
@@ -288,8 +308,13 @@
     }
     if (arith_mask & (1 << ARITH_F16)) {
         static const PackJobs jobsh = build_jobs_split(PACKH, PACKH.stream, 2);
-        hipLaunchKernelGGL(packh_kernel, dim3(8, jobsh.n), dim3(256), 0, stream, params, packed, jobsh);
-        hipLaunchKernelGGL(packth_small_kernel, dim3(11), dim3(256), 0, stream, params, packed);
+        if (fuse_f16) {
+            hipLaunchKernelGGL(pack_f16_kernel, dim3(PACKH_BLOCKS_PER_JOB * jobsh.n + PACK_SMALL_BLOCKS + PACKTH_SMALL_BLOCKS), dim3(256),
+                               0, stream, params, packed, jobsh);
+        } else {
+            hipLaunchKernelGGL(packh_kernel, dim3(PACKH_BLOCKS_PER_JOB, jobsh.n), dim3(256), 0, stream, params, packed, jobsh);
+            hipLaunchKernelGGL(packth_small_kernel, dim3(PACKTH_SMALL_BLOCKS), dim3(256), 0, stream, params, packed);
+        }
     }
     return hipGetLastError() == hipSuccess ? 0 : -3;
 }
diff --git a/dynhor_amd/fields.py b/dynhor_amd/fields.py
--- a/dynhor_amd/fields.py
+++ b/dynhor_amd/fields.py
@@ -151,8 +151,11 @@
             self._packed_sets = have
         return self.packed
 
+    def raw_inv_s(self) -> torch.Tensor:
+        return torch.exp(self.flat[self.var_off:self.var_off + 1] * 10.0)
+
     def inv_s(self) -> torch.Tensor:
-        return torch.exp(self.flat[self.var_off:self.var_off + 1] * 10.0).clip(1e-6, 1e6)
+        return self.raw_inv_s().clip(1e-6, 1e6)
 
     def adam_step(self, lr: float, betas=(0.9, 0.999), eps=1e-8, grad: torch.Tensor | None = None, grad_scale=1.0):
         g = grad if grad is not None else self.grad_flat
diff --git a/dynhor_amd/renderer.py b/dynhor_amd/renderer.py
--- a/dynhor_amd/renderer.py
+++ b/dynhor_amd/renderer.py
@@ -219,7 +219,7 @@
         return (marching_cubes if method == "cubes" else marching_tetrahedra)(u, threshold, bound_min, bound_max)
 
     @torch.no_grad()
-    def sample_z(self, rays_o, rays_d, near, far, perturb_overwrite=-1, t_rand=None):
+    def sample_z(self, rays_o, rays_d, near, far, perturb_overwrite=-1, t_rand=None, with_midpoints=False):
         L = _lib.lib()
         packed = self.store.ensure_packed(self._arith())
         dev = rays_o.device
@@ -237,35 +237,54 @@
         _lib.check(L.dh_coarse_samples(_p(rays_o), _p(rays_d), _p(near), _p(far),
                                        _p(t_rand.contiguous().view(-1)) if t_rand is not None else _NULL,
                                        B, ns, _p(z), _p(pts), _lib.stream()))
+        sample_dist = 2.0 / self.n_samples
+        n_cur = ns
+        pts_mid = None
         if self.n_importance > 0:
+            steps = self.up_sample_steps
             sdf = torch.empty(B * ns, device=dev)
             self._net_sdf_nograd("sdf_nograd_coarse", pts, B * ns, sdf)
-            n_new = self.n_importance // self.up_sample_steps
-            n_cur = ns
-            for i in range(self.up_sample_steps):
-                last = (i + 1 == self.up_sample_steps)
-                z_new = torch.empty(B, n_new, device=dev)
-                pts_new = torch.empty(B * n_new, 3, device=dev)
-                _lib.check(L.dh_upsample_step(_p(rays_o), _p(rays_d), _p(z), _p(sdf), B, n_cur, n_new,
-                                              float(64 * 2 ** i), _p(z_new), _p(pts_new), _lib.stream()))
+            n_new = self.n_importance // steps
+            z_new = torch.empty(B, n_new, device=dev)
+            pts_new = torch.empty(B * n_new, 3, device=dev)
+            _lib.check(L.dh_upsample_step(_p(rays_o), _p(rays_d), _p(z), _p(sdf), B, n_cur, n_new, 64.0, _p(z_new), _p(pts_new),
+                                          _lib.stream()))
+            for i in range(1, steps):
+                sdf_new = torch.empty(B * n_new, device=dev)
+                self._net_sdf_nograd("sdf_nograd_fine", pts_new, B * n_new, sdf_new)
+                inv_s = float(64 * 2 ** i)
+                if i + 1 < steps:
+                    z_out = torch.empty(B, n_cur + n_new, device=dev)
+                    sdf_out = torch.empty(B * (n_cur + n_new), device=dev)
+                    z_next = torch.empty(B, n_new, device=dev)
+                    pts_next = torch.empty(B * n_new, 3, device=dev)
+                    _lib.check(L.dh_merge_upsample_step(_p(rays_o), _p(rays_d), _p(z), _p(z_new), _p(sdf), _p(sdf_new), B, n_cur,
+                                                        n_new, n_new, inv_s, _p(z_out), _p(sdf_out), _p(z_next), _p(pts_next),
+                                                        _lib.stream()))
+                    z, sdf, z_new, pts_new = z_out, sdf_out, z_next, pts_next
+                    n_cur += n_new
+                else:
+                    z_out = torch.empty(B, n_cur + 2 * n_new, device=dev)
+                    pts_mid = torch.empty(B * (n_cur + 2 * n_new), 3, device=dev)
+                    _lib.check(L.dh_sample_tail(_p(rays_o), _p(rays_d), _p(z), _p(z_new), _p(sdf), _p(sdf_new), B, n_cur, n_new,
+                                                n_new, inv_s, sample_dist, _p(z_out), _p(pts_mid), _lib.stream()))
+                    z = z_out
+                    n_cur += 2 * n_new
+            if steps == 1:
                 z_out = torch.empty(B, n_cur + n_new, device=dev)
-                if not last:
-                    sdf_new = torch.empty(B * n_new, device=dev)
-                    self._net_sdf_nograd("sdf_nograd_fine", pts_new, B * n_new, sdf_new)
-                    sdf_out = torch.empty(B * (n_cur + n_new), device=dev)
-                    _lib.check(L.dh_merge_samples(_p(z), _p(z_new), _p(sdf), _p(sdf_new), B, n_cur, n_new, _p(z_out),
-                                                  _p(sdf_out), _lib.stream()))
-                    sdf = sdf_out
-                else:
-                    _lib.check(L.dh_merge_samples(_p(z), _p(z_new), _NULL, _NULL, B, n_cur, n_new, _p(z_out), _NULL,
-                                                  _lib.stream()))
+                _lib.check(L.dh_merge_samples(_p(z), _p(z_new), _NULL, _NULL, B, n_cur, n_new, _p(z_out), _NULL, _lib.stream()))
                 z = z_out
                 n_cur += n_new
-        return z
+        if not with_midpoints:
+            return z
+        if pts_mid is None:
+            pts_mid = torch.empty(B * n_cur, 3, device=dev)
+            _lib.check(L.dh_midpoints(_p(rays_o), _p(rays_d), _p(z), B, n_cur, sample_dist, _p(pts_mid), _lib.stream()))
+        return z, pts_mid
 
     @torch.no_grad()
     def _forward_core(self, rays_o, rays_d, z_vals, cos_anneal_ratio, background_rgb, want_nmap, infer_only=False,
-                      ray_grads=False):
+                      ray_grads=False, pts=None):
         L = _lib.lib()
         st = self.store
         packed = st.ensure_packed(self._arith())
@@ -280,13 +299,19 @@
         s.ray_grads = bool(ray_grads) and not infer_only
         self._ws_token += 1
         s.ws_token = self._ws_token
-        s.pts = torch.empty(P, 3, device=dev)
         s.sdf = torch.empty(P, device=dev)
         s.normals = torch.empty(P, 3, device=dev)
         s.colors = torch.empty(P, 3, device=dev)
-        _lib.check(L.dh_midpoints(_p(rays_o), _p(rays_d), _p(z_vals), B, n, s.sample_dist, _p(s.pts), _lib.stream()))
+        if pts is not None:
+            if pts.shape != (P, 3) or pts.dtype != torch.float32 or not pts.is_contiguous():
+                raise ValueError("pts must be the contiguous fp32 [B*n, 3] mid-points of z_vals")
+            s.pts = pts
+        else:
+            s.pts = torch.empty(P, 3, device=dev)
+            _lib.check(L.dh_midpoints(_p(rays_o), _p(rays_d), _p(z_vals), B, n, s.sample_dist, _p(s.pts), _lib.stream()))
         self._net_forward(s, packed)
-        s.inv_s = st.inv_s()
+        s.raw_inv_s = st.raw_inv_s()
+        s.inv_s = s.raw_inv_s.clip(1e-6, 1e6)
         s.weights = torch.empty(B, n, device=dev)
         s.color = torch.empty(B, 3, device=dev)
         s.wsum = torch.empty(B, 1, device=dev)
@@ -334,9 +359,7 @@
             d_sdf = (d_sdf + d_sdf_out.reshape(-1)).contiguous()
         grad = st.grad_bucket() if persistent else torch.empty(st.n, device=dev)
         self._net_backward(s, d_sdf, d_normals, d_colors, grad)
-        raw = torch.exp(st.flat[st.var_off] * 10.0)
-        passthrough = ((raw >= 1e-6) & (raw <= 1e6)).float()
-        grad[st.var_off] = d_inv_s.sum() * 10.0 * raw * passthrough
+        _lib.check(L.dh_variance_grad(_p(d_inv_s), B, _p(s.raw_inv_s), _p(grad), st.var_off, _lib.stream()))
         st.grad_flat = grad
         if s.ray_grads:
             dz = torch.cat([s.z_vals[:, 1:] - s.z_vals[:, :-1], torch.full_like(s.z_vals[:, :1], s.sample_dist)], -1)
@@ -384,9 +407,11 @@
         B = rays.shape[0]
         rays_o = rays[:, 0:3].contiguous()
         rays_d = rays[:, 3:6].contiguous()
-        z_vals = self.sample_z(rays_o, rays_d, near, far, t_rand=t_rand)
+        sampled = self.sample_z(rays_o, rays_d, near, far, t_rand=t_rand, with_midpoints=True)
+        z_vals, pts = sampled if isinstance(sampled, tuple) else (sampled, None)
         bg = None if background_rgb is None else background_rgb.reshape(-1).contiguous().float()
-        s = self._forward_core(rays_o, rays_d, z_vals, cos_anneal_ratio, bg, want_nmap=normal_weight > 0.0, ray_grads=ray_grads)
+        s = self._forward_core(rays_o, rays_d, z_vals, cos_anneal_ratio, bg, want_nmap=normal_weight > 0.0, ray_grads=ray_grads,
+                               pts=pts)
         stats = torch.empty(8, device=dev)
         d_color = torch.empty(B, 3, device=dev)
         d_wsum = torch.empty(B, device=dev)
diff --git a/include/dynhor_hip.h b/include/dynhor_hip.h
--- a/include/dynhor_hip.h
+++ b/include/dynhor_hip.h
@@ -97,6 +97,14 @@
 
 int dh_midpoints(const float* rays_o, const float* rays_d, const float* z, int64_t B, int n, float sample_dist, float* pts,
                  void* stream);
+
+int dh_merge_upsample_step(const float* rays_o, const float* rays_d, const float* z, const float* z_new, const float* sdf,
+                           const float* sdf_new, int64_t B, int n_cur, int n_new, int n_next, float inv_s, float* z_out,
+                           float* sdf_out, float* z_next, float* pts_next, void* stream);
+
+int dh_sample_tail(const float* rays_o, const float* rays_d, const float* z, const float* z_new, const float* sdf,
+                   const float* sdf_new, int64_t B, int n_cur, int n_new, int n_next, float inv_s, float sample_dist,
+                   float* z_vals, float* pts, void* stream);
 
 int dh_render_scan_fwd(const float* rays_o, const float* rays_d, const float* z, const float* sdf, const float* normals,
                        const float* colors, const float* inv_s, float cos_anneal_ratio, float sample_dist,
@@ -146,6 +154,8 @@
 int dh_adam_step(float* params, const float* grad, float* exp_avg, float* exp_avg_sq, int64_t n, float lr, float beta1,
                  float beta2, float eps, int64_t step, float grad_scale, void* stream);
 
+int dh_variance_grad(const float* d_inv_s, int64_t B, const float* raw, float* grad, int64_t var_off, void* stream);
+
 int64_t dh_hashgrid_entries(void);
 int dh_hashgrid_level(int level, float* scale, uint32_t* resolution, uint32_t* offset, uint32_t* dense);
 int dh_hashgrid_encode(const float* table, const float* x01, int64_t n, float* out, void* stream);
```

Result: no change. 231,700 rays/s, median of 6 (+0.6%).
